# cwchenwang/outdoor-nerf-depth

Hardware: AMD Instinct MI355X
Metric: train rays/sec, KITTI 375x1242, 64+128 samples/ray (higher is better)
Workload: dtype bf16 MFMA operands, f32 accumulate / f32 master weights

## Files before the change

include/nerfpp_hip.h:

```cpp
#ifndef NERFPP_HIP_H
#define NERFPP_HIP_H

#include <stdint.h>

#ifdef __cplusplus
extern "C" {
#endif

#define NERFPP_ABI_VERSION 9

#define NERFPP_OK 0
#define NERFPP_ERR_ARG 1
#define NERFPP_ERR_HIP 2
#define NERFPP_ERR_INTERNAL 3
#define NERFPP_ERR_UNSUPPORTED 4
#define NERFPP_ERR_COMM 5
#define NERFPP_ERR_LAUNCH NERFPP_ERR_HIP

#define NERFPP_PREC_BF16 1
#define NERFPP_PREC_SPLIT_BF16 2
#define NERFPP_PREC_FP16X2W 3

#define NERFPP_LOSS_RGB_ONLY 0
#define NERFPP_LOSS_MSE 1
#define NERFPP_LOSS_L1 2
#define NERFPP_LOSS_KL 3

#define NERFPP_FG_PARAMS 595844
#define NERFPP_BG_PARAMS 606596
#define NERFPP_LEVEL_PARAMS 1202440
#define NERFPP_MAX_SAMPLES 256

const char* nerfpp_last_error(void);
int nerfpp_abi_version(void);


int nerfpp_intersect_sphere(void* stream, int n_rays, const float* ray_o, const float* ray_d,
                            float* fg_far, int* bad_count);

int nerfpp_sample_coarse(void* stream, int n_rays, int n_samples, const float* ray_o,
                         const float* ray_d, const float* min_depth, const float* t_rand_fg,
                         const float* t_rand_bg, float* fg_far, float* fg_z, float* bg_z,
                         int* bad_count);

int nerfpp_sample_coarse_rng(void* stream, int n_rays, int n_samples, const float* ray_o,
                             const float* ray_d, const float* min_depth, uint64_t seed, uint64_t step,
                             float* fg_far, float* fg_z, float* bg_z, int* bad_count);

int nerfpp_rng_uniform(void* stream, uint64_t seed, uint64_t step, int stream_id, int64_t n, float* out);

int nerfpp_perturb_samples(void* stream, int n_rays, int n_samples, const float* z_vals,
                           const float* t_rand, float* out);

int nerfpp_sample_pdf(void* stream, int n_rays, int n_bins_m, int n_new, const float* bins,
                      const float* weights, const float* u, float* samples, int64_t* above_inds);

int nerfpp_sample_fine(void* stream, int n_rays, int s_old, int n_new, const float* z_old,
                       const float* weights, const float* u, float* z_merged, float* samples,
                       int64_t* above_inds);

int nerfpp_sample_fine_pair(void* stream, int n_rays, int s_old, int n_new, const float* fg_z_old,
                            const float* fg_weights, const float* fg_u, float* fg_z_merged,
                            const float* bg_z_old, const float* bg_weights, const float* bg_u,
                            float* bg_z_merged);

int nerfpp_sample_fine_pair_rng(void* stream, int n_rays, int s_old, int n_new, const float* fg_z_old,
                                const float* fg_weights, float* fg_z_merged, const float* bg_z_old,
                                const float* bg_weights, float* bg_z_merged, uint64_t seed, uint64_t step);

int nerfpp_sample_pixels(void* stream, uint64_t seed, uint64_t step, int64_t n_pixels, int n_rays, int64_t* pix);

int nerfpp_gather_rays(void* stream, int n_rays, int width, const float* cam, const int64_t* pix,
                       const float* rgb_img, const float* depth_img, float* ray_o, float* ray_d,
                       float* rgb, float* depth_sup, float* min_depth);


int nerfpp_table_sizes(int net, int64_t* fwd_elems, int64_t* fwd_bias_elems, int64_t* bwd_elems,
                       int64_t* slab_floats, int64_t* n_params);
int nerfpp_build_tables(int net, int32_t* fwd_tbl, int32_t* bias_tbl, int32_t* bwd_tbl,
                        int32_t* unpack_tbl);
int64_t nerfpp_level_tables_elems(void);
int nerfpp_build_level_tables(int32_t* host_tables);

int nerfpp_dw_plan(int64_t rows, int backward_precision, int32_t* k_out, int32_t* is_full_out);

int64_t nerfpp_packed_bytes(int precision);
int nerfpp_pack_level(void* stream, int precision, const float* params, const int32_t* tables,
                      void* packed);


int64_t nerfpp_workspace_bytes(int n_rays, int n_samples, int precision, int training);

int nerfpp_workspace_tensor(int n_rays, int n_samples, int precision, int net, int tensor,
                            int64_t* byte_offset, int32_t* ld, int64_t* plane_bytes);

typedef struct {
  int32_t n_rays, n_samples;
  int32_t precision, training;
  const float* ray_o;
  const float* ray_d;
  const float* fg_far;
  const float* fg_z;
  const float* bg_z;
  const void* packed;
  void* workspace;
  float* rgb;
  float* depth;
  float* fg_weights;
  float* bg_weights;
  float* fg_dists;
  float* fg_rgb;
  float* fg_depth;
  float* bg_rgb;
  float* bg_depth;
  float* bg_lambda;
  void* ev_mlp_begin;
  void* ev_mlp_end;
} nerfpp_forward_args;

int nerfpp_level_forward(void* stream, const nerfpp_forward_args* args);

int nerfpp_loss(void* stream, int n_rays, int n_samples, int loss_type, float lambda_depth,
                float kl_sigma, const float* rgb, const float* rgb_gt, const float* depth,
                const float* depth_sup, const float* fg_weights, const float* fg_z,
                const float* fg_dists, const float* fg_far, float* scalars, float* g_rgb,
                float* g_depth, float* g_fg_weights);

typedef struct {
  int32_t n_rays, n_samples;
  int32_t precision;
  int32_t workspace_precision;
  const float* ray_d;
  const float* fg_far;
  const float* fg_z;
  const float* bg_z;
  const void* packed;
  void* workspace;
  const int32_t* tables;
  const float* g_rgb;
  const float* g_depth;
  const float* g_fg_weights;
  float grad_scale;
  float* grads;
  void* ev_bwd_begin;
  void* ev_bwd_end;
  void* ev_dw_begin;
  void* ev_dw_end;
  const float* params;
  int32_t defer_reduce;
  int32_t fused_loss;
  int32_t loss_type;
  float lambda_depth;
  float kl_sigma;
  const float* rgb;
  const float* depth;
  const float* rgb_gt;
  const float* depth_sup;
  const int32_t* bad_count;
} nerfpp_backward_args;

int nerfpp_level_backward(void* stream, const nerfpp_backward_args* args);

int nerfpp_level_reduce_grads(void* stream, const nerfpp_backward_args* args);

int nerfpp_adam_step(void* stream, float* params, const float* grads, float* exp_avg,
                     float* exp_avg_sq, int64_t n, int step, double lr, double beta1, double beta2,
                     double eps, const float* skip_if_nonzero);

const char* nerfpp_comm_last_error(void);
int nerfpp_rccl_unique_id(char out_id[128]);
int nerfpp_rccl_comm_init(void** comm, int world_size, const char id[128], int rank);
int nerfpp_rccl_comm_destroy(void* comm);
int nerfpp_allreduce_mean(void* stream, void* rccl_comm, float* grads, int64_t count, int world_size, int prescaled);

int64_t nerfpp_image_metrics_workspace_bytes(int n_frames, int H, int W);
int nerfpp_image_metrics_u8(void* stream, int n_frames, int H, int W, const uint8_t* gt, const uint8_t* pred,
                            void* workspace, double* out);

#ifdef __cplusplus
}
#endif
#endif
```

outdoor_nerf_depth_amd/_lib.py:

```python
import ctypes as C
import os

from . import _ctypes_util as U

_HERE = os.path.dirname(os.path.abspath(__file__))
LIB_PATH = os.environ.get('NERFPP_HIP_LIB') or os.path.join(_HERE, 'libnerfpp_hip.so')

OK = 0
ABI_VERSION = 9
PREC_BF16, PREC_SPLIT_BF16 = 1, 2
PREC_FP16_FWD = 3
PREC_SPLIT_FWD = 12
LOSS_RGB_ONLY, LOSS_MSE, LOSS_L1, LOSS_KL = 0, 1, 2, 3
LOSS_TYPES = {'rgbonly': LOSS_RGB_ONLY, 'mse': LOSS_MSE, 'l1': LOSS_L1, 'kl': LOSS_KL}
FG_PARAMS, BG_PARAMS, LEVEL_PARAMS = 595844, 606596, 1202440
MAX_SAMPLES = 256

_fp = C.c_void_p
_i64p = C.POINTER(C.c_int64)
_i32p = C.POINTER(C.c_int32)


class ForwardArgs(C.Structure):
    _fields_ = [('n_rays', C.c_int32), ('n_samples', C.c_int32), ('precision', C.c_int32),
                ('training', C.c_int32)] + \
               [(k, _fp) for k in ('ray_o', 'ray_d', 'fg_far', 'fg_z', 'bg_z', 'packed', 'workspace',
                                   'rgb', 'depth', 'fg_weights', 'bg_weights', 'fg_dists', 'fg_rgb',
                                   'fg_depth', 'bg_rgb', 'bg_depth', 'bg_lambda', 'ev_mlp_begin',
                                   'ev_mlp_end')]


class BackwardArgs(C.Structure):
    _fields_ = [('n_rays', C.c_int32), ('n_samples', C.c_int32), ('precision', C.c_int32),
                ('workspace_precision', C.c_int32)] + \
               [(k, _fp) for k in ('ray_d', 'fg_far', 'fg_z', 'bg_z', 'packed', 'workspace', 'tables',
                                   'g_rgb', 'g_depth', 'g_fg_weights')] + \
               [('grad_scale', C.c_float), ('grads', _fp)] + \
               [(k, _fp) for k in ('ev_bwd_begin', 'ev_bwd_end', 'ev_dw_begin', 'ev_dw_end', 'params')] + \
               [('defer_reduce', C.c_int32), ('fused_loss', C.c_int32), ('loss_type', C.c_int32),
                ('lambda_depth', C.c_float), ('kl_sigma', C.c_float)] + \
               [(k, _fp) for k in ('rgb', 'depth', 'rgb_gt', 'depth_sup', 'bad_count')]


SYMBOLS = {
    'nerfpp_last_error': (C.c_char_p, []),
    'nerfpp_abi_version': (C.c_int, []),
    'nerfpp_intersect_sphere': (C.c_int, [_fp, C.c_int, _fp, _fp, _fp, _fp]),
    'nerfpp_sample_coarse': (C.c_int, [_fp, C.c_int, C.c_int] + [_fp] * 9),
    'nerfpp_sample_coarse_rng': (C.c_int, [_fp, C.c_int, C.c_int, _fp, _fp, _fp, C.c_uint64, C.c_uint64, _fp, _fp, _fp, _fp]),
    'nerfpp_rng_uniform': (C.c_int, [_fp, C.c_uint64, C.c_uint64, C.c_int, C.c_int64, _fp]),
    'nerfpp_sample_pixels': (C.c_int, [_fp, C.c_uint64, C.c_uint64, C.c_int64, C.c_int, _fp]),
    'nerfpp_perturb_samples': (C.c_int, [_fp, C.c_int, C.c_int, _fp, _fp, _fp]),
    'nerfpp_sample_pdf': (C.c_int, [_fp, C.c_int, C.c_int, C.c_int, _fp, _fp, _fp, _fp, _fp]),
    'nerfpp_sample_fine': (C.c_int, [_fp, C.c_int, C.c_int, C.c_int, _fp, _fp, _fp, _fp, _fp, _fp]),
    'nerfpp_sample_fine_pair': (C.c_int, [_fp, C.c_int, C.c_int, C.c_int, _fp, _fp, _fp, _fp, _fp, _fp, _fp, _fp]),
    'nerfpp_sample_fine_pair_rng': (C.c_int, [_fp, C.c_int, C.c_int, C.c_int, _fp, _fp, _fp, _fp, _fp, _fp, C.c_uint64,
                                              C.c_uint64]),
    'nerfpp_gather_rays': (C.c_int, [_fp, C.c_int, C.c_int] + [_fp] * 9),
    'nerfpp_table_sizes': (C.c_int, [C.c_int, _i64p, _i64p, _i64p, _i64p, _i64p]),
    'nerfpp_build_tables': (C.c_int, [C.c_int, _i32p, _i32p, _i32p, _i32p]),
    'nerfpp_level_tables_elems': (C.c_int64, []),
    'nerfpp_build_level_tables': (C.c_int, [_i32p]),
    'nerfpp_dw_plan': (C.c_int, [C.c_int64, C.c_int, _i32p, _i32p]),
    'nerfpp_packed_bytes': (C.c_int64, [C.c_int]),
    'nerfpp_pack_level': (C.c_int, [_fp, C.c_int, _fp, _fp, _fp]),
    'nerfpp_workspace_bytes': (C.c_int64, [C.c_int, C.c_int, C.c_int, C.c_int]),
    'nerfpp_workspace_tensor': (C.c_int, [C.c_int, C.c_int, C.c_int, C.c_int, C.c_int, _i64p, _i32p, _i64p]),
    'nerfpp_level_forward': (C.c_int, [_fp, C.POINTER(ForwardArgs)]),
    'nerfpp_loss': (C.c_int, [_fp, C.c_int, C.c_int, C.c_int, C.c_float, C.c_float] + [_fp] * 12),
    'nerfpp_level_backward': (C.c_int, [_fp, C.POINTER(BackwardArgs)]),
    'nerfpp_level_reduce_grads': (C.c_int, [_fp, C.POINTER(BackwardArgs)]),
    'nerfpp_adam_step': (C.c_int, [_fp, _fp, _fp, _fp, _fp, C.c_int64, C.c_int, C.c_double, C.c_double,
                                   C.c_double, C.c_double, _fp]),
    'nerfpp_image_metrics_workspace_bytes': (C.c_int64, [C.c_int, C.c_int, C.c_int]),
    'nerfpp_image_metrics_u8': (C.c_int, [_fp, C.c_int, C.c_int, C.c_int, _fp, _fp, _fp, _fp]),
    'nerfpp_comm_last_error': (C.c_char_p, []),
    'nerfpp_rccl_unique_id': (C.c_int, [C.c_char_p]),
    'nerfpp_rccl_comm_init': (C.c_int, [C.POINTER(C.c_void_p), C.c_int, C.c_char_p, C.c_int]),
    'nerfpp_rccl_comm_destroy': (C.c_int, [_fp]),
    'nerfpp_allreduce_mean': (C.c_int, [_fp, _fp, _fp, C.c_int64, C.c_int, C.c_int]),
}

_lib = None


class NerfppError(RuntimeError):
    pass


def lib():
    global _lib
    if _lib is None:
        _lib = U.load(LIB_PATH, 'libnerfpp_hip.so', SYMBOLS, 'nerfpp_abi_version', ABI_VERSION, NerfppError,
                      ' (hipcc --offload-arch=gfx950). There is no CPU fallback for the NeRF++ hot path.')
    return _lib


check = U.checker(lib, 'nerfpp_last_error', NerfppError, 'nerfpp call')


def build_level_tables():
    import numpy as np
    n = lib().nerfpp_level_tables_elems()
    out = np.empty(n, np.int32)
    check(lib().nerfpp_build_level_tables(out.ctypes.data_as(_i32p)), 'nerfpp_build_level_tables')
    return out


def build_net_tables(net):
    import numpy as np
    sizes = [C.c_int64() for _ in range(5)]
    check(lib().nerfpp_table_sizes(net, *[C.byref(s) for s in sizes]), 'nerfpp_table_sizes')
    fwd, bias, bwd, slab, npar = [s.value for s in sizes]
    arrs = [np.empty(n, np.int32) for n in (fwd, bias, bwd, npar)]
    check(lib().nerfpp_build_tables(net, *[a.ctypes.data_as(_i32p) for a in arrs]), 'nerfpp_build_tables')
    return arrs[0], arrs[1], arrs[2], arrs[3], slab
```

outdoor_nerf_depth_amd/csrc/nerfpp_api.hip:

```cpp
#include "probe_env.h"
#include <hip/hip_runtime.h>
#include <stdio.h>
#include <stdlib.h>
#include <string.h>
#include "../../include/nerfpp_hip.h"
#define API_OK NERFPP_OK
#define API_ERR_HIP NERFPP_ERR_HIP
#define API_ERR_ARG NERFPP_ERR_ARG
#include "api_common.h"
#include "nerfpp_common.h"
#include "nerfpp_kernels.h"

using namespace nerfpp;

namespace {

constexpr size_t align_up(size_t v, size_t a) { return (v + a - 1) / a * a; }
bool h0_recomputed(int WP) { return a_planes(WP) == 1; }

struct TblLayout { int64_t fwd[2], bias[2], bwd[2], unpack[2], total; };
TblLayout tbl_layout() {
  TblLayout L{};
  int64_t off = 0;
  for (int net = 0; net < N_NET; ++net) {
    L.fwd[net] = off; off += (int64_t)fwd_frags(net) * 512;
    L.bias[net] = off; off += FWD_BIAS_FLOATS;
    L.bwd[net] = off; off += (int64_t)BWD_FRAGS * 512;
    L.unpack[net] = off; off += net_params(net);
  }
  L.total = off;
  return L;
}

struct PackLayout { size_t fwd[2], bwd[2], bias[2], derived[2], total; };
PackLayout pack_layout(int P) {
  PackLayout L{};
  size_t off = 0;
  for (int net = 0; net < N_NET; ++net) {
    L.fwd[net] = off; off = align_up(off + fwd_stream_bytes(net, P), 256);
    L.bwd[net] = off; off = align_up(off + bwd_stream_bytes(P), 256);
    L.bias[net] = off; off = align_up(off + FWD_BIAS_FLOATS * sizeof(float), 256);
    L.derived[net] = off; off = align_up(off + DERIVED_FLOATS * sizeof(float), 256);
  }
  L.total = off;
  return L;
}

struct WsLayout {
  size_t tensor[2][T_COUNT], out_raw[2], depth_real, d_out[2], slabs[2], masks[2], fix_m[2], total;
  int64_t rows, rows_padded;
  int ksplit;
};
int choose_ksplit(int64_t rows) {
  int k = 1;
  for (int rc = 0; rc < 2; ++rc) {
    const DwPlan pl = dw_plan(rows, rc != 0);
    for (int net = 0; net < N_NET; ++net)
      for (int j = 0; j < DW_JOBS; ++j) k = pl.k[net][j] > k ? pl.k[net][j] : k;
  }
  return k;
}
WsLayout ws_layout(int n_rays, int S, int P, bool training) {
  WsLayout L{};
  L.rows = (int64_t)n_rays * S;
  L.rows_padded = (int64_t)align_up((size_t)L.rows, 256);
  L.ksplit = choose_ksplit(L.rows);
  size_t off = 0;
  for (int net = 0; net < N_NET; ++net) {
    L.out_raw[net] = off; off = align_up(off + (size_t)L.rows_padded * 16, 256);
    if (training) {
      L.d_out[net] = off; off = align_up(off + (size_t)L.rows_padded * 16, 256);
      for (int t = 0; t < T_COUNT; ++t) {
        L.tensor[net][t] = off;
        if (t == T_R || t == T_DR) continue;
        if (t == T_DG) continue;
        if (t == T_H0 && h0_recomputed(P)) continue;
        if (t == T_DZ0 + 7 && h0_recomputed(P)) continue;
        off = align_up(off + (size_t)L.rows_padded * tensor_ld(net, t) * 2 * a_planes(P), 256);
      }
      L.slabs[net] = off; off = align_up(off + (size_t)L.ksplit * gslab_floats(net) * 4, 256);
      L.masks[net] = off; off = align_up(off + (size_t)9 * (L.rows_padded / 32) * 64 * 16, 256);
      L.fix_m[net] = off; off = align_up(off + (size_t)128 * 256 * 4, 256);
    }
  }
  L.depth_real = off; off = align_up(off + (size_t)L.rows_padded * 4, 256);
  L.total = off;
  return L;
}

NetWs make_netws(char* ws, const WsLayout& L, int net) {
  NetWs w;
  for (int t = 0; t < T_COUNT; ++t) w.t[t] = (__bf16*)(ws + L.tensor[net][t]);
  w.t[T_DG] = w.t[T_DS] + (DG_COL0 / 16) * (FRAG_BYTES / 2);
  return w;
}

bool prec_ok(int P) { return P == NERFPP_PREC_BF16 || P == NERFPP_PREC_SPLIT_BF16; }
bool prec_ok_fwd(int P) { return prec_ok(P) || P == NERFPP_PREC_FP16X2W; }

bool split_nets() {
  static const bool on = PROBE_GETENV("NERFPP_MLP_SPLIT") != nullptr;
  return on;
}

}

extern "C" {

const char* nerfpp_last_error(void) { return g_err; }
int nerfpp_abi_version(void) { return NERFPP_ABI_VERSION; }

int nerfpp_intersect_sphere(void* stream, int n_rays, const float* ray_o, const float* ray_d, float* fg_far,
                            int* bad_count) {
  REQUIRE(n_rays > 0 && ray_o && ray_d && fg_far, "non-null inputs, n_rays > 0");
  launch_intersect_sphere((hipStream_t)stream, n_rays, ray_o, ray_d, fg_far, bad_count);
  return check_launch("intersect_sphere");
}

int nerfpp_sample_coarse(void* stream, int n_rays, int n_samples, const float* ray_o, const float* ray_d,
                         const float* min_depth, const float* t_rand_fg, const float* t_rand_bg, float* fg_far,
                         float* fg_z, float* bg_z, int* bad_count) {
  REQUIRE(n_rays > 0 && n_samples >= 2 && n_samples <= NERFPP_MAX_SAMPLES, "2 <= n_samples <= 256");
  REQUIRE(ray_o && ray_d && min_depth && fg_far && fg_z && bg_z, "non-null pointers");
  launch_sample_coarse((hipStream_t)stream, n_rays, n_samples, ray_o, ray_d, min_depth, t_rand_fg, t_rand_bg,
                       fg_far, fg_z, bg_z, bad_count, make_rng_key(0, 0, false));
  return check_launch("sample_coarse");
}

int nerfpp_sample_coarse_rng(void* stream, int n_rays, int n_samples, const float* ray_o, const float* ray_d,
                             const float* min_depth, uint64_t seed, uint64_t step, float* fg_far, float* fg_z,
                             float* bg_z, int* bad_count) {
  REQUIRE(n_rays > 0 && n_samples >= 2 && n_samples <= NERFPP_MAX_SAMPLES, "2 <= n_samples <= 256");
  REQUIRE(ray_o && ray_d && min_depth && fg_far && fg_z && bg_z, "non-null pointers");
  launch_sample_coarse((hipStream_t)stream, n_rays, n_samples, ray_o, ray_d, min_depth, nullptr, nullptr, fg_far,
                       fg_z, bg_z, bad_count, make_rng_key(seed, step, true));
  return check_launch("sample_coarse_rng");
}

int nerfpp_rng_uniform(void* stream, uint64_t seed, uint64_t step, int stream_id, int64_t n, float* out) {
  REQUIRE(n > 0 && out && stream_id >= 0 && stream_id <= 3, "stream_id in 0..3, non-null output");
  launch_rng_uniform((hipStream_t)stream, make_rng_key(seed, step, true), (uint32_t)stream_id, n, out);
  return check_launch("rng_uniform");
}

int nerfpp_perturb_samples(void* stream, int n_rays, int n_samples, const float* z_vals, const float* t_rand,
                           float* out) {
  REQUIRE(n_rays > 0 && n_samples >= 2 && z_vals && t_rand && out, "non-null pointers");
  launch_perturb((hipStream_t)stream, n_rays, n_samples, z_vals, t_rand, out);
  return check_launch("perturb_samples");
}

int nerfpp_sample_pdf(void* stream, int n_rays, int n_bins_m, int n_new, const float* bins, const float* weights,
                      const float* u, float* samples, int64_t* above_inds) {
  REQUIRE(n_rays > 0 && n_bins_m >= 1 && n_bins_m + 1 <= 512 && n_new >= 1 && n_new <= 512, "sizes");
  REQUIRE(bins && weights && samples, "non-null pointers");
  launch_sample_pdf((hipStream_t)stream, false, n_rays, n_bins_m, n_new, bins, weights, u, samples, above_inds,
                    nullptr);
  return check_launch("sample_pdf");
}

int nerfpp_sample_fine(void* stream, int n_rays, int s_old, int n_new, const float* z_old, const float* weights,
                       const float* u, float* z_merged, float* samples, int64_t* above_inds) {
  REQUIRE(n_rays > 0 && s_old >= 3 && n_new >= 1 && s_old + n_new <= 512, "3 <= s_old, s_old + n_new <= 512");
  REQUIRE(z_old && weights && z_merged, "non-null pointers");
  launch_sample_pdf((hipStream_t)stream, true, n_rays, s_old - 2, n_new, z_old, weights, u, samples, above_inds,
                    z_merged);
  return check_launch("sample_fine");
}

int nerfpp_sample_fine_pair(void* stream, int n_rays, int s_old, int n_new, const float* fg_z_old,
                            const float* fg_weights, const float* fg_u, float* fg_z_merged, const float* bg_z_old,
                            const float* bg_weights, const float* bg_u, float* bg_z_merged) {
  REQUIRE(n_rays > 0 && s_old >= 3 && n_new >= 1 && s_old + n_new <= 512, "3 <= s_old, s_old + n_new <= 512");
  REQUIRE(fg_z_old && fg_weights && fg_z_merged && bg_z_old && bg_weights && bg_z_merged, "non-null pointers");
  const float* z[2] = {fg_z_old, bg_z_old};
  const float* w[2] = {fg_weights, bg_weights};
  const float* u[2] = {fg_u, bg_u};
  float* m[2] = {fg_z_merged, bg_z_merged};
  launch_sample_fine_pair((hipStream_t)stream, n_rays, s_old - 2, n_new, z, w, u, m, make_rng_key(0, 0, false));
  return check_launch("sample_fine_pair");
}

int nerfpp_sample_fine_pair_rng(void* stream, int n_rays, int s_old, int n_new, const float* fg_z_old,
                                const float* fg_weights, float* fg_z_merged, const float* bg_z_old,
                                const float* bg_weights, float* bg_z_merged, uint64_t seed, uint64_t step) {
  REQUIRE(n_rays > 0 && s_old >= 3 && n_new >= 1 && s_old + n_new <= 512, "3 <= s_old, s_old + n_new <= 512");
  REQUIRE(fg_z_old && fg_weights && fg_z_merged && bg_z_old && bg_weights && bg_z_merged, "non-null pointers");
  const float* z[2] = {fg_z_old, bg_z_old};
  const float* w[2] = {fg_weights, bg_weights};
  const float* u[2] = {nullptr, nullptr};
  float* m[2] = {fg_z_merged, bg_z_merged};
  launch_sample_fine_pair((hipStream_t)stream, n_rays, s_old - 2, n_new, z, w, u, m, make_rng_key(seed, step, true));
  return check_launch("sample_fine_pair_rng");
}

int nerfpp_sample_pixels(void* stream, uint64_t seed, uint64_t step, int64_t n_pixels, int n_rays, int64_t* pix) {
  REQUIRE(pix && n_rays >= 1 && n_rays <= 8192, "1 <= n_rays <= 8192, non-null output");
  REQUIRE(n_pixels >= n_rays && n_pixels < ((int64_t)1 << 31), "n_rays <= n_pixels < 2^31");
  launch_sample_pixels((hipStream_t)stream, make_rng_key(seed, step, true), n_pixels, n_rays, pix);
  return check_launch("sample_pixels");
}

int nerfpp_gather_rays(void* stream, int n_rays, int width, const float* cam, const int64_t* pix,
                       const float* rgb_img, const float* depth_img, float* ray_o, float* ray_d, float* rgb,
                       float* depth_sup, float* min_depth) {
  REQUIRE(n_rays > 0 && width > 0 && cam && pix && ray_o && ray_d && min_depth, "non-null pointers");
  REQUIRE((rgb == nullptr) || rgb_img, "rgb output needs rgb_img");
  REQUIRE((depth_sup == nullptr) || depth_img, "depth_sup output needs depth_img");
  launch_gather_rays((hipStream_t)stream, n_rays, width, cam, pix, rgb_img, depth_img, ray_o, ray_d, rgb, depth_sup,
                     min_depth);
  return check_launch("gather_rays");
}

int64_t nerfpp_level_tables_elems(void) { return tbl_layout().total; }

int nerfpp_build_level_tables(int32_t* host_tables) {
  if (!host_tables) return fail(NERFPP_ERR_ARG, "nerfpp_build_level_tables: null buffer");
  const TblLayout L = tbl_layout();
  for (int net = 0; net < N_NET; ++net) {
    const int rc = nerfpp_build_tables(net, host_tables + L.fwd[net], host_tables + L.bias[net],
                                       host_tables + L.bwd[net], host_tables + L.unpack[net]);
    if (rc != NERFPP_OK) return fail(rc, "nerfpp_build_tables(%d) failed", net);
  }
  return NERFPP_OK;
}

int nerfpp_dw_plan(int64_t rows, int backward_precision, int32_t* k_out, int32_t* is_full_out) {
  if (!k_out || rows <= 0 || !prec_ok(backward_precision)) return -1;
  const DwPlan pl = dw_plan(rows, backward_precision == 1);
  const JobTable jt = build_all_jobs();
  for (int net = 0; net < N_NET; ++net)
    for (int j = 0; j < DW_JOBS; ++j) {
      k_out[net * DW_JOBS + j] = pl.k[net][j];
      if (is_full_out) is_full_out[net * DW_JOBS + j] = dw_job_is_full(jt.jobs[net][j]) ? 1 : 0;
    }
  return DW_JOBS;
}

int64_t nerfpp_packed_bytes(int precision) { return prec_ok_fwd(precision) ? (int64_t)pack_layout(precision).total : -1; }

int nerfpp_pack_level(void* stream, int precision, const float* params, const int32_t* tables, void* packed) {
  REQUIRE(prec_ok_fwd(precision), "precision must be 1, 2 or 3");
  REQUIRE(params && tables && packed, "non-null pointers");
  const TblLayout T = tbl_layout();
  const PackLayout L = pack_layout(precision);
  hipStream_t st = (hipStream_t)stream;
  char* out = (char*)packed;
  const int32_t* tbl[3 * N_NET];
  void* outs[3 * N_NET];
  int64_t n[3 * N_NET];
  for (int net = 0; net < N_NET; ++net) {
    tbl[3 * net] = tables + T.fwd[net];      outs[3 * net] = out + L.fwd[net];      n[3 * net] = (int64_t)fwd_frags(net) * 512;
    tbl[3 * net + 1] = tables + T.bwd[net];  outs[3 * net + 1] = out + L.bwd[net];  n[3 * net + 1] = (int64_t)BWD_FRAGS * 512;
    tbl[3 * net + 2] = tables + T.bias[net]; outs[3 * net + 2] = out + L.bias[net]; n[3 * net + 2] = FWD_BIAS_FLOATS;
  }
  float* derived[N_NET] = {(float*)(out + L.derived[0]), (float*)(out + L.derived[1])};
  launch_pack_level(st, params, precision, tbl, outs, n, derived);
  return check_launch("pack_level");
}

int64_t nerfpp_workspace_bytes(int n_rays, int n_samples, int precision, int training) {
  if (n_rays <= 0 || n_samples < 2 || n_samples > NERFPP_MAX_SAMPLES || !prec_ok_fwd(precision)) return -1;
  return (int64_t)ws_layout(n_rays, n_samples, precision, training != 0).total;
}

int nerfpp_workspace_tensor(int n_rays, int n_samples, int precision, int net, int tensor, int64_t* byte_offset,
                            int32_t* ld, int64_t* plane_bytes) {
  REQUIRE(n_rays > 0 && n_samples >= 2 && n_samples <= NERFPP_MAX_SAMPLES && prec_ok_fwd(precision), "sizes / precision");
  REQUIRE(net >= 0 && net < N_NET && tensor >= 0 && tensor < T_COUNT && tensor != T_R && tensor != T_DR, "net / tensor id");
  REQUIRE(byte_offset && ld && plane_bytes, "non-null outputs");
  if (tensor == T_H0 && h0_recomputed(precision))
    return fail(NERFPP_ERR_UNSUPPORTED, "nerfpp_workspace_tensor: H0 is not materialised at precision %d (its weight-gradient job recomputes it from X)", precision);
  if (tensor == T_DZ0 + 7 && h0_recomputed(precision))
    return fail(NERFPP_ERR_UNSUPPORTED, "nerfpp_workspace_tensor: dZ7 is not materialised at precision %d (its weight-gradient job recomputes it from [dS | dG])", precision);
  const WsLayout L = ws_layout(n_rays, n_samples, precision, true);
  const int l = tensor_ld(net, tensor);
  *byte_offset = tensor == T_DG ? (int64_t)L.tensor[net][T_DS] + (DG_COL0 / 16) * FRAG_BYTES : (int64_t)L.tensor[net][tensor];
  *ld = l;
  *plane_bytes = (int64_t)L.rows_padded * l * 2;
  return NERFPP_OK;
}

int nerfpp_level_forward(void* stream, const nerfpp_forward_args* a) {
  REQUIRE(a, "args");
  REQUIRE(a->n_rays > 0 && a->n_samples >= 2 && a->n_samples <= NERFPP_MAX_SAMPLES, "sizes");
  REQUIRE(prec_ok_fwd(a->precision), "precision must be 1, 2 or 3");
  REQUIRE(a->ray_o && a->ray_d && a->fg_far && a->fg_z && a->bg_z && a->packed && a->workspace, "inputs");
  REQUIRE(a->rgb && a->depth && a->fg_weights && a->bg_weights && a->fg_dists && a->fg_rgb && a->fg_depth &&
          a->bg_rgb && a->bg_depth && a->bg_lambda, "outputs");
  hipStream_t st = (hipStream_t)stream;
  const int P = a->precision;
  const bool train = a->training != 0;
  const WsLayout L = ws_layout(a->n_rays, a->n_samples, P, train);
  const PackLayout PL = pack_layout(P);
  char* ws = (char*)a->workspace;
  const char* pk = (const char*)a->packed;
  MlpFwdArgs mm[N_NET];
  for (int net = 0; net < N_NET; ++net) {
    MlpFwdArgs& m = mm[net];
    m = MlpFwdArgs{};
    m.geom.ray_o = a->ray_o;
    m.geom.ray_d = a->ray_d;
    m.geom.z = net == 0 ? a->fg_z : a->bg_z;
    m.rows = L.rows;
    m.rows_padded = L.rows_padded;
    m.S = a->n_samples;
    m.w_stream = pk + PL.fwd[net];
    m.bias = (const float*)(pk + PL.bias[net]);
    m.out_raw = (float*)(ws + L.out_raw[net]);
    m.depth_real = (float*)(ws + L.depth_real);
    if (train) { m.ws = make_netws(ws, L, net); m.masks = (uint4*)(ws + L.masks[net]); }
    m.save_lo = a->training == 2 ? 0 : 1;
    m.skip_h0 = (train && (h0_recomputed(P) || a->training == 2)) ? 1 : 0;
  }
  if (a->ev_mlp_begin) (void)hipEventRecord((hipEvent_t)a->ev_mlp_begin, st);
  if (split_nets()) {
    launch_mlp_fwd_pair(st, P, train, mm[0], mm[1], 1);
    launch_mlp_fwd_pair(st, P, train, mm[0], mm[1], 2);
  } else {
    launch_mlp_fwd_pair(st, P, train, mm[0], mm[1], 0);
  }
  if (a->ev_mlp_end) (void)hipEventRecord((hipEvent_t)a->ev_mlp_end, st);
  launch_composite_fwd(st, a->n_rays, a->n_samples, (const float*)(ws + L.out_raw[0]),
                       (const float*)(ws + L.out_raw[1]), (const float*)(ws + L.depth_real), a->ray_d, a->fg_far,
                       a->fg_z, a->bg_z, a->rgb, a->depth, a->fg_weights, a->bg_weights, a->fg_dists, a->fg_rgb,
                       a->fg_depth, a->bg_rgb, a->bg_depth, a->bg_lambda);
  return check_launch("level_forward");
}

int nerfpp_loss(void* stream, int n_rays, int n_samples, int loss_type, float lambda_depth, float kl_sigma,
                const float* rgb, const float* rgb_gt, const float* depth, const float* depth_sup,
                const float* fg_weights, const float* fg_z, const float* fg_dists, const float* fg_far,
                float* scalars, float* g_rgb, float* g_depth, float* g_fg_weights) {
  REQUIRE(n_rays > 0 && loss_type >= 0 && loss_type <= 3, "loss_type in 0..3");
  REQUIRE(rgb && rgb_gt && scalars && g_rgb && g_depth, "non-null pointers");
  if (loss_type != NERFPP_LOSS_RGB_ONLY) REQUIRE(depth && depth_sup, "depth loss needs depth and depth_sup");
  if (loss_type == NERFPP_LOSS_KL)
    REQUIRE(fg_weights && fg_z && fg_dists && fg_far && g_fg_weights && kl_sigma > 0.f, "KL inputs");
  launch_loss((hipStream_t)stream, n_rays, n_samples, loss_type, lambda_depth, kl_sigma, rgb, rgb_gt, depth,
              depth_sup, fg_weights, fg_z, fg_dists, fg_far, scalars, g_rgb, g_depth, g_fg_weights);
  return check_launch("loss");
}

}

static void weight_grads(hipStream_t st, const nerfpp_backward_args* a, const WsLayout& L) {
  char* ws = (char*)a->workspace;
  DwArgs dw{};
  for (int net = 0; net < N_NET; ++net) {
    dw.ws[net] = make_netws(ws, L, net);
    dw.slabs[net] = (float*)(ws + L.slabs[net]);
  }
  dw.rows = L.rows;
  dw.rows_padded = L.rows_padded;
  dw.h0_from_x = a->precision == 1 ? 1 : 0;
  const PackLayout PL = pack_layout(a->precision);
  for (int net = 0; net < N_NET; ++net) {
    dw.fwd_w[net] = (const char*)a->packed + PL.fwd[net];
    dw.fwd_bias[net] = (const float*)((const char*)a->packed + PL.bias[net]);
    dw.bwd_w[net] = (const char*)a->packed + PL.bwd[net];
    dw.masks[net] = (const uint4*)(ws + L.masks[net]);
  }
  dw.plan = dw_plan(L.rows, dw.h0_from_x != 0);
  if (a->ev_dw_begin) (void)hipEventRecord((hipEvent_t)a->ev_dw_begin, st);
  launch_dw(st, a->precision, dw);
  if (a->ev_dw_end) (void)hipEventRecord((hipEvent_t)a->ev_dw_end, st);
}
static bool defer_dw() {
  static const bool on = PROBE_GETENV("NERFPP_DEFER_DW") != nullptr;
  return on;
}

static void reduce_grads(hipStream_t st, const nerfpp_backward_args* a, const WsLayout& L, const TblLayout& T) {
  char* ws = (char*)a->workspace;
  const DwPlan plan = dw_plan(L.rows, a->precision == 1);
  const float* slabs[N_NET];
  int64_t slab_floats[N_NET];
  const int32_t* utbl[N_NET];
  float* m_out[N_NET];
  for (int net = 0; net < N_NET; ++net) {
    slabs[net] = (const float*)(ws + L.slabs[net]);
    slab_floats[net] = gslab_floats(net);
    utbl[net] = a->tables + T.unpack[net];
    m_out[net] = (float*)(ws + L.fix_m[net]);
  }
  static const int skip = PROBE_GETENV("NERFPP_REDUCE_SKIP") ? atoi(PROBE_GETENV("NERFPP_REDUCE_SKIP")) : 0;
  if (!(skip & 1)) launch_unpack_grads(st, slabs, slab_floats, plan, utbl, m_out, a->grad_scale, a->grads, a->bad_count);
  if (!(skip & 2)) launch_remap_fixup(st, a->grads, a->params, m_out[0], m_out[1]);
}

extern "C" {

int nerfpp_level_reduce_grads(void* stream, const nerfpp_backward_args* a) {
  REQUIRE(a, "args");
  REQUIRE(a->n_rays > 0 && a->n_samples >= 2 && a->n_samples <= NERFPP_MAX_SAMPLES, "sizes");
  REQUIRE(prec_ok(a->precision), "precision must be 1 or 2");
  REQUIRE(a->workspace && a->tables && a->grads && a->params, "workspace / tables / grads / params");
  const int WP = a->workspace_precision ? a->workspace_precision : a->precision;
  REQUIRE(prec_ok_fwd(WP) && a_planes(WP) >= a_planes(a->precision), "workspace_precision: 0, or a forward precision that saved the planes this backward reads");
  const WsLayout L = ws_layout(a->n_rays, a->n_samples, WP, true);
  if (defer_dw()) weight_grads((hipStream_t)stream, a, L);
  reduce_grads((hipStream_t)stream, a, L, tbl_layout());
  return check_launch("level_reduce_grads");
}

int nerfpp_level_backward(void* stream, const nerfpp_backward_args* a) {
  REQUIRE(a, "args");
  REQUIRE(a->n_rays > 0 && a->n_samples >= 2 && a->n_samples <= NERFPP_MAX_SAMPLES, "sizes");
  REQUIRE(prec_ok(a->precision), "precision must be 1 or 2");
  REQUIRE(a->ray_d && a->fg_far && a->fg_z && a->bg_z && a->packed && a->workspace && a->tables, "inputs");
  REQUIRE(a->grads && a->params, "gradients / params");
  LossFuse lf{};
  if (a->fused_loss) {
    REQUIRE(a->loss_type >= NERFPP_LOSS_RGB_ONLY && a->loss_type <= NERFPP_LOSS_KL, "loss_type in 0..3");
    REQUIRE(a->rgb && a->rgb_gt, "fused loss head needs rgb and rgb_gt");
    if (a->loss_type != NERFPP_LOSS_RGB_ONLY) REQUIRE(a->depth && a->depth_sup, "fused depth loss needs depth and depth_sup");
    if (a->loss_type == NERFPP_LOSS_KL) REQUIRE(a->kl_sigma > 0.f, "kl_sigma > 0");
    lf.type = a->loss_type; lf.lambda_depth = a->lambda_depth; lf.kl_sigma = a->kl_sigma;
    lf.rgb = a->rgb; lf.depth = a->depth; lf.rgb_gt = a->rgb_gt; lf.depth_sup = a->depth_sup;
  } else {
    REQUIRE(a->g_rgb && a->g_depth, "dL/d rgb and dL/d depth (or fused_loss)");
  }
  hipStream_t st = (hipStream_t)stream;
  const int P = a->precision;
  const int WP = a->workspace_precision ? a->workspace_precision : P;
  REQUIRE(prec_ok_fwd(WP) && a_planes(WP) >= a_planes(P), "workspace_precision: 0, or a forward precision that saved the planes this backward reads");
  const WsLayout L = ws_layout(a->n_rays, a->n_samples, WP, true);
  const PackLayout PL = pack_layout(P);
  const TblLayout T = tbl_layout();
  char* ws = (char*)a->workspace;
  const char* pk = (const char*)a->packed;
  launch_composite_bwd(st, a->n_rays, a->n_samples, (const float*)(ws + L.out_raw[0]),
                       (const float*)(ws + L.out_raw[1]), (const float*)(ws + L.depth_real), a->ray_d, a->fg_far,
                       a->fg_z, a->bg_z, a->g_rgb, a->g_depth, a->g_fg_weights, (float*)(ws + L.d_out[0]),
                       (float*)(ws + L.d_out[1]), a->fused_loss ? &lf : nullptr);
  MlpBwdArgs mb[N_NET];
  for (int net = 0; net < N_NET; ++net) {
    MlpBwdArgs& m = mb[net];
    m = MlpBwdArgs{};
    m.rows = L.rows;
    m.rows_padded = L.rows_padded;
    m.w_stream = pk + PL.bwd[net];
    m.d_out = (const float*)(ws + L.d_out[net]);
    m.ws = make_netws(ws, L, net);
    m.masks = (const uint4*)(ws + L.masks[net]);
    m.skip_dz7 = P == 1 ? 1 : 0;
  }
  if (a->ev_bwd_begin) (void)hipEventRecord((hipEvent_t)a->ev_bwd_begin, st);
  if (split_nets()) {
    launch_mlp_bwd_pair(st, P, mb[0], mb[1], 1);
    launch_mlp_bwd_pair(st, P, mb[0], mb[1], 2);
  } else {
    launch_mlp_bwd_pair(st, P, mb[0], mb[1], 0);
  }
  if (a->ev_bwd_end) (void)hipEventRecord((hipEvent_t)a->ev_bwd_end, st);
  if (!(a->defer_reduce && defer_dw())) weight_grads(st, a, L);
  if (!a->defer_reduce) reduce_grads(st, a, L, T);
  return check_launch("level_backward");
}

int nerfpp_adam_step(void* stream, float* params, const float* grads, float* exp_avg, float* exp_avg_sq,
                     int64_t n, int step, double lr, double beta1, double beta2, double eps,
                     const float* skip_if_nonzero) {
  REQUIRE(params && grads && exp_avg && exp_avg_sq && n > 0 && step >= 1, "non-null pointers, step >= 1");
  launch_adam((hipStream_t)stream, params, grads, exp_avg, exp_avg_sq, n, step, lr, beta1, beta2, eps, skip_if_nonzero);
  return check_launch("adam_step");
}

static int image_metrics_sizes_ok(const char* fn, int n_frames, int H, int W) {
  if (n_frames < 1 || n_frames > 65535) return fail(NERFPP_ERR_ARG, "%s: n_frames = %d, expected 1 .. 65535", fn, n_frames);
  if (H < 7 || W < 7)
    return fail(NERFPP_ERR_ARG, "%s: a %d x %d image is smaller than the 7 x 7 SSIM window (H >= 7 and W >= 7)", fn, H, W);
  if (H > 32768 || W > 32768) return fail(NERFPP_ERR_ARG, "%s: a %d x %d image exceeds 32768 pixels per side", fn, H, W);
  return NERFPP_OK;
}

int64_t nerfpp_image_metrics_workspace_bytes(int n_frames, int H, int W) {
  if (image_metrics_sizes_ok(__func__, n_frames, H, W) != NERFPP_OK) return -1;
  return (int64_t)n_frames * image_metrics_tiles(H, W) * 4 * 8;
}

int nerfpp_image_metrics_u8(void* stream, int n_frames, int H, int W, const uint8_t* gt, const uint8_t* pred,
                            void* workspace, double* out) {
  const int rc = image_metrics_sizes_ok(__func__, n_frames, H, W);
  if (rc != NERFPP_OK) return rc;
  REQUIRE(gt && pred && workspace && out, "non-null gt, pred, workspace, out");
  REQUIRE(((uintptr_t)workspace & 7) == 0 && ((uintptr_t)out & 7) == 0, "workspace and out aligned to 8 bytes");
  launch_image_metrics((hipStream_t)stream, n_frames, H, W, gt, pred, workspace, out);
  return check_launch("image_metrics_u8");
}

}
```

outdoor_nerf_depth_amd/csrc/nerfpp_kernels.h:

```cpp
#pragma once
#include <hip/hip_runtime.h>
#include <stdint.h>
#include "nerfpp_common.h"

namespace nerfpp {

struct MlpGeom {
  const float* ray_o;
  const float* ray_d;
  const float* z;
};

struct NetWs {
  __bf16* t[T_COUNT];
};

struct MlpFwdArgs {
  MlpGeom geom;
  int64_t rows, rows_padded;
  int S;
  const void* w_stream;
  const float* bias;
  float* out_raw;
  float* depth_real;
  NetWs ws;
  uint4* masks;
  int save_lo;
  int skip_h0;
};

struct MlpBwdArgs {
  int64_t rows, rows_padded;
  const void* w_stream;
  const float* d_out;
  NetWs ws;
  const uint4* masks;
  int skip_dz7;
};

struct LossFuse {
  int type;
  float lambda_depth, kl_sigma;
  const float* rgb;
  const float* depth;
  const float* rgb_gt;
  const float* depth_sup;
};

struct DwArgs {
  NetWs ws[N_NET];
  int64_t rows, rows_padded;
  float* slabs[N_NET];
  DwPlan plan;
  int h0_from_x;
  const void* fwd_w[N_NET];
  const float* fwd_bias[N_NET];
  const void* bwd_w[N_NET];
  const uint4* masks[N_NET];
};

}

void launch_intersect_sphere(hipStream_t st, int n, const float* o, const float* d, float* far, int* bad);
void launch_sample_coarse(hipStream_t st, int n, int S, const float* o, const float* d, const float* min_depth,
                          const float* t_fg, const float* t_bg, float* far, float* fg_z, float* bg_z, int* bad,
                          const nerfpp::RngKey& rng);
void launch_rng_uniform(hipStream_t st, const nerfpp::RngKey& rng, uint32_t stream_id, int64_t n, float* out);
void launch_perturb(hipStream_t st, int n, int S, const float* z, const float* t, float* out);
void launch_sample_pdf(hipStream_t st, bool fused, int n, int M, int S_new, const float* bins_or_zold,
                       const float* weights, const float* u, float* samples, int64_t* above, float* merged);
void launch_sample_fine_pair(hipStream_t st, int n, int M, int S_new, const float* const* z_old,
                             const float* const* weights, const float* const* u, float* const* merged,
                             const nerfpp::RngKey& rng);
void launch_composite_fwd(hipStream_t st, int n, int S, const float* raw_fg, const float* raw_bg,
                          const float* depth_real_bg, const float* ray_d, const float* fg_far,
                          const float* fg_z, const float* bg_z, float* rgb, float* depth, float* fg_weights,
                          float* bg_weights, float* fg_dists, float* fg_rgb, float* fg_depth, float* bg_rgb,
                          float* bg_depth, float* bg_lambda);
void launch_composite_bwd(hipStream_t st, int n, int S, const float* raw_fg, const float* raw_bg,
                          const float* depth_real_bg, const float* ray_d, const float* fg_far,
                          const float* fg_z, const float* bg_z, const float* g_rgb, const float* g_depth,
                          const float* g_fg_weights, float* dout_fg, float* dout_bg, const nerfpp::LossFuse* lf);
void launch_loss(hipStream_t st, int n, int S, int type, float lambda_depth, float kl_sigma, const float* rgb,
                 const float* rgb_gt, const float* depth, const float* depth_sup, const float* fg_weights,
                 const float* fg_z, const float* fg_dists, const float* fg_far, float* scalars, float* g_rgb,
                 float* g_depth, float* g_fg_weights);
int launch_sample_pixels(hipStream_t st, const nerfpp::RngKey& rng, int64_t n_pixels, int k, int64_t* pix);
void launch_gather_rays(hipStream_t st, int n, int W, const float* cam, const int64_t* pix, const float* rgb_img,
                        const float* depth_img, float* ray_o, float* ray_d, float* rgb, float* depth_sup,
                        float* min_depth);
void launch_mlp_fwd_pair(hipStream_t st, int P, bool train, const nerfpp::MlpFwdArgs& a_fg, const nerfpp::MlpFwdArgs& a_bg, int which);
void launch_mlp_bwd_pair(hipStream_t st, int P, const nerfpp::MlpBwdArgs& a_fg, const nerfpp::MlpBwdArgs& a_bg, int which);
void launch_dw(hipStream_t st, int P, const nerfpp::DwArgs& a);
void launch_pack_level(hipStream_t st, const float* params, int P, const int32_t* const* tbl, void* const* out,
                       const int64_t* n, float* const* derived);
void launch_unpack_grads(hipStream_t st, const float* const* slabs, const int64_t* slab_floats,
                         const nerfpp::DwPlan& plan, const int32_t* const* tbl, float* const* m_out, float scale,
                         float* grads_lvl, const int32_t* bad_count);
void launch_remap_fixup(hipStream_t st, float* grads_lvl, const float* params_lvl, const float* m0, const float* m1);
void launch_adam(hipStream_t st, float* p, const float* g, float* m, float* v, int64_t n, int step, double lr,
                 double beta1, double beta2, double eps, const float* skip);
int64_t image_metrics_tiles(int H, int W);
void launch_image_metrics(hipStream_t st, int F, int H, int W, const unsigned char* gt, const unsigned char* pred,
                          void* workspace, double* out);
```

outdoor_nerf_depth_amd/csrc/nerfpp_render.hip:

```cpp
#include <hip/hip_runtime.h>
#include <math.h>
#include <stdint.h>
#include "hip_device.h"
#include "nerfpp_common.h"
#include "nerfpp_kernels.h"

namespace nerfpp {

using hipdev::wave_sum, hipdev::wave_excl_suffix_sum, hipdev::lds_tree_sum;

constexpr float TINY = 1e-6f;
constexpr float HUGE_NUM = 1e10f;

__device__ __forceinline__ float sum3(float a, float b, float c) { return (a + b) + c; }

__device__ __forceinline__ float sphere_far(const float* __restrict__ ray_o,
                                            const float* __restrict__ ray_d, int ray, int* bad) {
  const float ox = ray_o[ray * 3], oy = ray_o[ray * 3 + 1], oz = ray_o[ray * 3 + 2];
  const float dx = ray_d[ray * 3], dy = ray_d[ray * 3 + 1], dz = ray_d[ray * 3 + 2];
  const float dd = sum3(dx * dx, dy * dy, dz * dz);
  const float d1 = -sum3(dx * ox, dy * oy, dz * oz) / dd;
  const float px = ox + d1 * dx, py = oy + d1 * dy, pz = oz + d1 * dz;
  const float ray_d_cos = 1.f / sqrtf(dd);
  const float pn = sum3(px * px, py * py, pz * pz);
  if (pn >= 1.f && bad) atomicAdd(bad, 1);
  const float d2 = sqrtf(1.f - pn) * ray_d_cos;
  return d1 + d2;
}

__global__ void intersect_sphere_kernel(int n, const float* __restrict__ ray_o,
                                        const float* __restrict__ ray_d, float* __restrict__ far,
                                        int* bad) {
  const int ray = blockIdx.x * blockDim.x + threadIdx.x;
  if (ray < n) far[ray] = sphere_far(ray_o, ray_d, ray, bad);
}

__device__ __forceinline__ float torch_linspace01(int i, int steps) {
  const float step = 1.f / (float)(steps - 1);
  return i < steps / 2 ? fmaf(step, (float)i, 0.f) : fmaf(-step, (float)(steps - 1 - i), 1.f);
}

__device__ __forceinline__ float perturb(float zm, float z0, float zp, bool first, bool last, float t) {
  const float upper = last ? z0 : .5f * (zp + z0);
  const float lower = first ? z0 : .5f * (z0 + zm);
  return lower + (upper - lower) * t;
}

__global__ void sample_coarse_kernel(int n, int S, const float* __restrict__ ray_o,
                                     const float* __restrict__ ray_d,
                                     const float* __restrict__ min_depth,
                                     const float* __restrict__ t_fg, const float* __restrict__ t_bg,
                                     float* __restrict__ fg_far, float* __restrict__ fg_z,
                                     float* __restrict__ bg_z, int* bad, RngKey rng) {
  const int idx = blockIdx.x * blockDim.x + threadIdx.x;
  if (idx >= n * S) return;
  const int ray = idx / S, i = idx - ray * S;
  const float far = sphere_far(ray_o, ray_d, ray, i == 0 ? bad : nullptr);
  if (i == 0) fg_far[ray] = far;
  const float near = min_depth[ray];
  const float step = (far - near) / (float)(S - 1);
  const float z0 = near + (float)i * step;
  float out = z0;
  if (t_fg || rng.enabled) {
    const float zm = near + (float)(i - 1) * step, zp = near + (float)(i + 1) * step;
    out = perturb(zm, z0, zp, i == 0, i == S - 1, rng.enabled ? philox_uniform(rng, 0, (uint64_t)idx) : t_fg[idx]);
  }
  fg_z[idx] = out;
  const float b0 = torch_linspace01(i, S);
  out = b0;
  if (t_bg || rng.enabled) {
    const float bm = i > 0 ? torch_linspace01(i - 1, S) : 0.f;
    const float bp = i < S - 1 ? torch_linspace01(i + 1, S) : 0.f;
    out = perturb(bm, b0, bp, i == 0, i == S - 1, rng.enabled ? philox_uniform(rng, 1, (uint64_t)idx) : t_bg[idx]);
  }
  bg_z[idx] = out;
}

__global__ void rng_uniform_kernel(RngKey rng, uint32_t stream_id, int64_t n, float* __restrict__ out) {
  const int64_t i = (int64_t)blockIdx.x * blockDim.x + threadIdx.x;
  if (i < n) out[i] = philox_uniform(rng, stream_id, (uint64_t)i);
}

__global__ void perturb_kernel(int n, int S, const float* __restrict__ z, const float* __restrict__ t,
                               float* __restrict__ out) {
  const int idx = blockIdx.x * blockDim.x + threadIdx.x;
  if (idx >= n * S) return;
  const int i = idx % S;
  const float z0 = z[idx];
  const float zm = i > 0 ? z[idx - 1] : 0.f, zp = i < S - 1 ? z[idx + 1] : 0.f;
  out[idx] = perturb(zm, z0, zp, i == 0, i == S - 1, t[idx]);
}

constexpr int SP_MAX = 512;
__device__ __forceinline__ void lds_wave_sync() {
  asm volatile("s_waitcnt lgkmcnt(0)" ::: "memory");
  __builtin_amdgcn_wave_barrier();
}

struct SamplePdfProblem {
  const float* bins_or_zold; const float* weights; const float* u;
  float* samples; int64_t* above; float* merged;
};
struct SamplePdfArgs { SamplePdfProblem p[2]; RngKey rng; };
template <bool FUSED>
__global__ __launch_bounds__(256) void sample_pdf_kernel(int n, int M, int S_new, SamplePdfArgs args) {
  const SamplePdfProblem& pr = args.p[blockIdx.y];
  const float* __restrict__ bins_or_zold = pr.bins_or_zold;
  const float* __restrict__ weights = pr.weights;
  const float* __restrict__ u_in = pr.u;
  float* __restrict__ samples_out = pr.samples;
  int64_t* __restrict__ above_out = pr.above;
  float* __restrict__ merged_out = pr.merged;
  __shared__ float s_cdf[4][SP_MAX];
  __shared__ float s_w[4][SP_MAX];
  __shared__ float s_bins[4][SP_MAX];
  __shared__ float s_z[4][SP_MAX];
  const int wave = threadIdx.x >> 6, lane = threadIdx.x & 63;
  const int ray = blockIdx.x * 4 + wave;
  const bool active = ray < n;
  const int S_old = FUSED ? M + 2 : 0;
  float* cdf = s_cdf[wave];
  float* wq = s_w[wave];
  float* bins = s_bins[wave];
  float* zs = s_z[wave];
  if (active) {
    if (FUSED) {
      const float* zo = bins_or_zold + (size_t)ray * S_old;
      for (int i = lane; i < S_old; i += 64) zs[i] = zo[i];
      for (int k = lane; k < M; k += 64) wq[k] = weights[(size_t)ray * S_old + k + 1] + TINY;
    } else {
      for (int i = lane; i <= M; i += 64) bins[i] = bins_or_zold[(size_t)ray * (M + 1) + i];
      for (int k = lane; k < M; k += 64) wq[k] = weights[(size_t)ray * M + k] + TINY;
    }
  }
  __syncthreads();
  if (active) {
    if (FUSED)
      for (int i = lane; i <= M; i += 64) bins[i] = .5f * (zs[i + 1] + zs[i]);
    if (lane == 0) {
      double acc = 0.0;
      for (int k = 0; k < M; ++k) acc += (double)wq[k];
      cdf[0] = (float)acc;
    }
  }
  __syncthreads();
  if (active) {
    const float wsum = cdf[0];
    for (int k = lane; k < M; k += 64) wq[k] = wq[k] / wsum;
  }
  __syncthreads();
  if (active && lane == 0) {
    double acc = 0.0;
    cdf[0] = 0.f;
    for (int k = 0; k < M; ++k) {
      acc += (double)wq[k];
      cdf[k + 1] = (float)acc;
    }
  }
  __syncthreads();
  if (active) {
    for (int j = lane; j < S_new; j += 64) {
      const float u = args.rng.enabled ? philox_uniform(args.rng, 2u + blockIdx.y, (uint64_t)ray * S_new + j)
                      : u_in ? u_in[(size_t)ray * S_new + j] : torch_linspace01(j, S_new);
      int above = 0, hi_ = M;
      while (above < hi_) {
        const int mid = (above + hi_) >> 1;
        const bool ge = u >= cdf[mid];
        above = ge ? mid + 1 : above;
        hi_ = ge ? hi_ : mid;
      }
      const int below = above - 1 > 0 ? above - 1 : 0;
      const float cdf_lo = cdf[below], cdf_hi = cdf[above];
      const float bin_lo = bins[below], bin_hi = bins[above];
      float denom = cdf_hi - cdf_lo;
      denom = denom < TINY ? 1.f : denom;
      const float t = (u - cdf_lo) / denom;
      const float s = bin_lo + t * (bin_hi - bin_lo + TINY);
      if (samples_out) samples_out[(size_t)ray * S_new + j] = s;
      if (above_out) above_out[(size_t)ray * S_new + j] = above;
      if (FUSED) zs[S_old + j] = s;
    }
  }
  if (!FUSED) return;
  __syncthreads();
  if (active && merged_out) {
    const int S_tot = S_old + S_new;
    bool sorted_old = true;
    for (int i = lane; i + 1 < S_old; i += 64) sorted_old = sorted_old && zs[i] <= zs[i + 1];
    if (__all(sorted_old) && S_new <= SP_MAX) {
      int P2 = 1;
      while (P2 < S_new) P2 <<= 1;
      float* nb = wq;
      for (int i = lane; i < P2; i += 64) nb[i] = i < S_new ? zs[S_old + i] : __builtin_inff();
      lds_wave_sync();
      for (int k = 2; k <= P2; k <<= 1) {
        for (int j = k >> 1; j > 0; j >>= 1) {
          for (int t = lane; t < (P2 >> 1); t += 64) {
            const int lo = ((t & ~(j - 1)) << 1) | (t & (j - 1)), hi_i = lo | j;
            const bool up = (lo & k) == 0;
            const float x = nb[lo], y = nb[hi_i];
            if ((x > y) == up) { nb[lo] = y; nb[hi_i] = x; }
          }
          lds_wave_sync();
        }
      }
      float* mo = merged_out + (size_t)ray * S_tot;
      for (int i = lane; i < S_old; i += 64) {
        const float v = zs[i];
        int lo = 0, hi_i = S_new;
        while (lo < hi_i) {
          const int mid = (lo + hi_i) >> 1;
          const bool lt = nb[mid] < v;
          lo = lt ? mid + 1 : lo;
          hi_i = lt ? hi_i : mid;
        }
        mo[i + lo] = v;
      }
      for (int p = lane; p < S_new; p += 64) {
        const float v = nb[p];
        int lo = 0, hi_i = S_old;
        while (lo < hi_i) {
          const int mid = (lo + hi_i) >> 1;
          const bool le = zs[mid] <= v;
          lo = le ? mid + 1 : lo;
          hi_i = le ? hi_i : mid;
        }
        mo[p + lo] = v;
      }
      return;
    }
    if (S_tot <= 192) {
      const int e0 = lane, e1 = lane + 64, e2 = lane + 128;
      const float v0 = e0 < S_tot ? zs[e0] : 0.f, v1 = e1 < S_tot ? zs[e1] : 0.f, v2 = e2 < S_tot ? zs[e2] : 0.f;
      int r0 = 0, r1 = 0, r2 = 0;
#pragma unroll 4
      for (int k = 0; k < S_tot; ++k) {
        const float o = zs[k];
        r0 += (o < v0 || (o == v0 && k < e0)) ? 1 : 0;
        r1 += (o < v1 || (o == v1 && k < e1)) ? 1 : 0;
        r2 += (o < v2 || (o == v2 && k < e2)) ? 1 : 0;
      }
      float* mo = merged_out + (size_t)ray * S_tot;
      if (e0 < S_tot) mo[r0] = v0;
      if (e1 < S_tot) mo[r1] = v1;
      if (e2 < S_tot) mo[r2] = v2;
      return;
    }
    for (int e = lane; e < S_tot; e += 64) {
      const float v = zs[e];
      int rank = 0;
      for (int k = 0; k < S_tot; ++k) {
        const float o = zs[k];
        rank += (o < v || (o == v && k < e)) ? 1 : 0;
      }
      merged_out[(size_t)ray * S_tot + rank] = v;
    }
  }
}

constexpr int CPL_MAX = 4;

__device__ __forceinline__ float wave_excl_prod(float x, int lane, float* total) {
  float v = x;
#pragma unroll
  for (int d = 1; d < 64; d <<= 1) {
    const float t = __shfl_up(v, d, 64);
    if (lane >= d) v *= t;
  }
  *total = __shfl(v, 63, 64);
  const float e = __shfl_up(v, 1, 64);
  return lane == 0 ? 1.f : e;
}

struct RaySamples {
  float dist[CPL_MAX], e[CPL_MAX], alpha[CPL_MAX], q[CPL_MAX], T[CPL_MAX], w[CPL_MAX];
  float c[CPL_MAX][3], zval[CPL_MAX], sraw[CPL_MAX];
  float lambda;
};

template <bool BG>
__device__ __forceinline__ void load_volume(RaySamples& v, int S, int cpl, int lane, size_t row0,
                                            const float4* __restrict__ raw, const float* __restrict__ z,
                                            const float* __restrict__ depth_real, float dnorm, float far) {
  float run = 1.f;
#pragma unroll
  for (int k = 0; k < CPL_MAX; ++k) {
    const int i = lane * cpl + k;
    const bool ok = k < cpl && i < S;
    float dist = 0.f, sraw = 0.f, zv = 0.f;
    float c0 = 0.f, c1 = 0.f, c2 = 0.f;
    if (ok) {
      const int s = BG ? S - 1 - i : i;
      const float4 r = raw[row0 + s];
      c0 = r.x; c1 = r.y; c2 = r.z; sraw = r.w;
      if (BG) {
        const float zi = z[s];
        dist = i < S - 1 ? zi - z[s - 1] : HUGE_NUM;
        zv = depth_real[row0 + s];
      } else {
        const float zi = z[i];
        dist = dnorm * ((i < S - 1 ? z[i + 1] : far) - zi);
        zv = zi;
      }
    }
    const float sigma = fabsf(sraw);
    const float e = ok ? expf(-sigma * dist) : 1.f;
    const float alpha = 1.f - e;
    const float q = ok ? 1.f - alpha + TINY : 1.f;
    v.dist[k] = dist; v.e[k] = e; v.alpha[k] = alpha; v.q[k] = q;
    v.c[k][0] = c0; v.c[k][1] = c1; v.c[k][2] = c2; v.zval[k] = zv; v.sraw[k] = sraw;
    v.T[k] = run;
    run *= q;
  }
  float total;
  const float pre = wave_excl_prod(run, lane, &total);
  v.lambda = total;
#pragma unroll
  for (int k = 0; k < CPL_MAX; ++k) {
    v.T[k] *= pre;
    v.w[k] = v.alpha[k] * v.T[k];
  }
}

__global__ __launch_bounds__(256) void composite_fwd_kernel(
    int n, int S, const float4* __restrict__ raw_fg, const float4* __restrict__ raw_bg,
    const float* __restrict__ depth_real_bg, const float* __restrict__ ray_d,
    const float* __restrict__ fg_far, const float* __restrict__ fg_z, const float* __restrict__ bg_z,
    float* __restrict__ rgb, float* __restrict__ depth, float* __restrict__ fg_weights,
    float* __restrict__ bg_weights, float* __restrict__ fg_dists, float* __restrict__ fg_rgb,
    float* __restrict__ fg_depth, float* __restrict__ bg_rgb, float* __restrict__ bg_depth,
    float* __restrict__ bg_lambda) {
  const int wave = threadIdx.x >> 6, lane = threadIdx.x & 63;
  const int ray = blockIdx.x * 4 + wave;
  if (ray >= n) return;
  const int cpl = (S + 63) / 64;
  const size_t row0 = (size_t)ray * S;
  const float dx = ray_d[ray * 3], dy = ray_d[ray * 3 + 1], dz = ray_d[ray * 3 + 2];
  const float dnorm = sqrtf(sum3(dx * dx, dy * dy, dz * dz));
  RaySamples v;
  load_volume<false>(v, S, cpl, lane, row0, raw_fg, fg_z + row0, nullptr, dnorm, fg_far[ray]);
  float a0 = 0, a1 = 0, a2 = 0, ad = 0;
#pragma unroll
  for (int k = 0; k < CPL_MAX; ++k) {
    const int i = lane * cpl + k;
    if (k < cpl && i < S) {
      fg_weights[row0 + i] = v.w[k];
      fg_dists[row0 + i] = v.dist[k];
      a0 += v.w[k] * v.c[k][0]; a1 += v.w[k] * v.c[k][1]; a2 += v.w[k] * v.c[k][2];
      ad += v.w[k] * v.zval[k];
    }
  }
  const float f0 = wave_sum(a0), f1 = wave_sum(a1), f2 = wave_sum(a2), fd = wave_sum(ad);
  const float lam = v.lambda;
  load_volume<true>(v, S, cpl, lane, row0, raw_bg, bg_z + row0, depth_real_bg, dnorm, 0.f);
  a0 = a1 = a2 = ad = 0;
#pragma unroll
  for (int k = 0; k < CPL_MAX; ++k) {
    const int i = lane * cpl + k;
    if (k < cpl && i < S) {
      bg_weights[row0 + i] = v.w[k];
      a0 += v.w[k] * v.c[k][0]; a1 += v.w[k] * v.c[k][1]; a2 += v.w[k] * v.c[k][2];
      ad += v.w[k] * v.zval[k];
    }
  }
  const float b0 = lam * wave_sum(a0), b1 = lam * wave_sum(a1), b2 = lam * wave_sum(a2);
  const float bd = lam * wave_sum(ad);
  if (lane == 0) {
    fg_rgb[ray * 3] = f0; fg_rgb[ray * 3 + 1] = f1; fg_rgb[ray * 3 + 2] = f2;
    bg_rgb[ray * 3] = b0; bg_rgb[ray * 3 + 1] = b1; bg_rgb[ray * 3 + 2] = b2;
    rgb[ray * 3] = f0 + b0; rgb[ray * 3 + 1] = f1 + b1; rgb[ray * 3 + 2] = f2 + b2;
    fg_depth[ray] = fd; bg_depth[ray] = bd; depth[ray] = fd + bd; bg_lambda[ray] = lam;
  }
}

struct KlFuse { bool on; float gt, inv2s, lambda_depth; };
template <bool BG>
__device__ __forceinline__ void volume_backward(const RaySamples& v, int S, int cpl, int lane, size_t row0,
                                                const float gC[3], float gD, float g_lam_lam,
                                                const float* __restrict__ g_w_extra,
                                                float4* __restrict__ dout, const KlFuse kl = KlFuse{false, 0.f, 0.f, 0.f}) {
  float gw[CPL_MAX], term = 0.f;
#pragma unroll
  for (int k = 0; k < CPL_MAX; ++k) {
    const int i = lane * cpl + k;
    const bool ok = k < cpl && i < S;
    float g = gC[0] * v.c[k][0] + gC[1] * v.c[k][1] + gC[2] * v.c[k][2] + gD * v.zval[k];
    if (ok && g_w_extra) g += g_w_extra[row0 + i];
    if (!BG && ok && kl.on) {
      const float dz = v.zval[k] - kl.gt;
      const float w = v.w[k] + 1e-5f;
      const float e = expf(-(dz * dz) * kl.inv2s);
      g += -kl.lambda_depth * e * v.dist[k] / (w * (float)S);
    }
    gw[k] = ok ? g : 0.f;
    term += gw[k] * v.w[k];
  }
  float suffix = wave_excl_suffix_sum(term, lane);
#pragma unroll
  for (int k = CPL_MAX - 1; k >= 0; --k) {
    const int i = lane * cpl + k;
    if (k < cpl && i < S) {
      const float d_a = gw[k] * v.T[k] - (suffix + g_lam_lam) / v.q[k];
      const float d_sigma = d_a * v.dist[k] * v.e[k];
      const float sgn = v.sraw[k] > 0.f ? 1.f : (v.sraw[k] < 0.f ? -1.f : 0.f);
      float4 o;
      o.x = v.w[k] * gC[0] * v.c[k][0] * (1.f - v.c[k][0]);
      o.y = v.w[k] * gC[1] * v.c[k][1] * (1.f - v.c[k][1]);
      o.z = v.w[k] * gC[2] * v.c[k][2] * (1.f - v.c[k][2]);
      o.w = d_sigma * sgn;
      const int s = BG ? S - 1 - i : i;
      dout[row0 + s] = o;
    }
    suffix += gw[k] * v.w[k];
  }
}

template <bool LF>
__global__ __launch_bounds__(256) void composite_bwd_kernel(
    int n, int S, const float4* __restrict__ raw_fg, const float4* __restrict__ raw_bg,
    const float* __restrict__ depth_real_bg, const float* __restrict__ ray_d,
    const float* __restrict__ fg_far, const float* __restrict__ fg_z, const float* __restrict__ bg_z,
    const float* __restrict__ g_rgb, const float* __restrict__ g_depth,
    const float* __restrict__ g_fg_weights, float4* __restrict__ dout_fg, float4* __restrict__ dout_bg, LossFuse lf) {
  const int wave = threadIdx.x >> 6, lane = threadIdx.x & 63;
  const int ray = blockIdx.x * 4 + wave;
  float cnt = 0.f;
  if (LF && (lf.type == 1 || lf.type == 2)) {
    __shared__ float s_cnt[4];
    float c = 0.f;
    for (int r = threadIdx.x; r < n; r += 256) c += lf.depth_sup[r] > 0.f ? 1.f : 0.f;
    c = wave_sum(c);
    if (lane == 0) s_cnt[wave] = c;
    __syncthreads();
    cnt = (s_cnt[0] + s_cnt[1]) + (s_cnt[2] + s_cnt[3]);
  }
  if (ray >= n) return;
  const int cpl = (S + 63) / 64;
  const size_t row0 = (size_t)ray * S;
  const float dx = ray_d[ray * 3], dy = ray_d[ray * 3 + 1], dz = ray_d[ray * 3 + 2];
  const float dnorm = sqrtf(sum3(dx * dx, dy * dy, dz * dz));
  float gC[3], gD;
  KlFuse kl{false, 0.f, 0.f, 0.f};
  if (LF) {
#pragma unroll
    for (int c = 0; c < 3; ++c) gC[c] = 2.f * (lf.rgb[ray * 3 + c] - lf.rgb_gt[ray * 3 + c]) / (float)(3 * n);
    gD = 0.f;
    if (lf.type == 1 || lf.type == 2) {
      const float gt = lf.depth_sup[ray];
      if (gt > 0.f && cnt > 0.f) {
        const float d = lf.depth[ray] - gt;
        gD = lf.type == 1 ? lf.lambda_depth * 2.f * d / cnt
                          : lf.lambda_depth * (d > 0.f ? 1.f : (d < 0.f ? -1.f : 0.f)) / cnt;
      }
    } else if (lf.type == 3) {
      const float gt = lf.depth_sup[ray];
      kl.on = gt > 0.f && gt < fg_far[ray];
      kl.gt = gt;
      kl.inv2s = 1.f / (2.f * lf.kl_sigma);
      kl.lambda_depth = lf.lambda_depth;
    }
  } else {
    gC[0] = g_rgb[ray * 3]; gC[1] = g_rgb[ray * 3 + 1]; gC[2] = g_rgb[ray * 3 + 2];
    gD = g_depth[ray];
  }
  RaySamples vb;
  load_volume<true>(vb, S, cpl, lane, row0, raw_bg, bg_z + row0, depth_real_bg, dnorm, 0.f);
  float a0 = 0, a1 = 0, a2 = 0, ad = 0;
#pragma unroll
  for (int k = 0; k < CPL_MAX; ++k) {
    a0 += vb.w[k] * vb.c[k][0]; a1 += vb.w[k] * vb.c[k][1]; a2 += vb.w[k] * vb.c[k][2];
    ad += vb.w[k] * vb.zval[k];
  }
  const float g_lam = gC[0] * wave_sum(a0) + gC[1] * wave_sum(a1) + gC[2] * wave_sum(a2) + gD * wave_sum(ad);
  RaySamples vf;
  load_volume<false>(vf, S, cpl, lane, row0, raw_fg, fg_z + row0, nullptr, dnorm, fg_far[ray]);
  const float lam = vf.lambda;
  volume_backward<false>(vf, S, cpl, lane, row0, gC, gD, g_lam * lam, LF ? nullptr : g_fg_weights, dout_fg, kl);
  const float gCb[3] = {lam * gC[0], lam * gC[1], lam * gC[2]};
  volume_backward<true>(vb, S, cpl, lane, row0, gCb, lam * gD, 0.f, nullptr, dout_bg);
}

__device__ double block_sum(double v, double (&sh)[1][1024]) {
  lds_tree_sum(sh, {v});
  const double r = sh[0][0];
  __syncthreads();
  return r;
}

__global__ __launch_bounds__(256) void kl_terms_kernel(
    int n, int S, float lambda_depth, float kl_sigma, const float* __restrict__ depth_sup,
    const float* __restrict__ fg_weights, const float* __restrict__ fg_z, const float* __restrict__ fg_dists,
    const float* __restrict__ fg_far, float* __restrict__ ray_sum, float* __restrict__ g_fg_weights) {
  const int wave = threadIdx.x >> 6, lane = threadIdx.x & 63;
  const int ray = blockIdx.x * 4 + wave;
  if (ray >= n) return;
  const float gt = depth_sup[ray];
  const bool m = gt > 0.f && gt < fg_far[ray];
  const float inv2s = 1.f / (2.f * kl_sigma);
  double acc = 0.0;
  for (int s = lane; s < S; s += 64) {
    const size_t i = (size_t)ray * S + s;
    float g = 0.f;
    if (m) {
      const float dz = fg_z[i] - gt;
      const float w = fg_weights[i] + 1e-5f;
      const float e = expf(-(dz * dz) * inv2s);
      acc += (double)(-logf(w) * e * fg_dists[i]);
      g = -lambda_depth * e * fg_dists[i] / (w * (float)S);
    }
    g_fg_weights[i] = g;
  }
  acc = wave_sum(acc);
  if (lane == 0) ray_sum[ray] = (float)acc;
}

__global__ __launch_bounds__(1024) void loss_kernel(
    int n, int S, int type, float lambda_depth, float kl_sigma, const float* __restrict__ rgb,
    const float* __restrict__ rgb_gt, const float* __restrict__ depth, const float* __restrict__ depth_sup,
    const float* __restrict__ fg_weights, const float* __restrict__ fg_z, const float* __restrict__ fg_dists,
    const float* __restrict__ fg_far, float* __restrict__ scalars, float* __restrict__ g_rgb,
    float* __restrict__ g_depth, float* __restrict__ g_fg_weights) {
  __shared__ double sh[1][1024];
  double s_rgb = 0, s_dep = 0, s_cnt = 0;
  for (int r = threadIdx.x; r < n; r += blockDim.x) {
    for (int c = 0; c < 3; ++c) {
      const float d = rgb[r * 3 + c] - rgb_gt[r * 3 + c];
      s_rgb += (double)(d * d);
    }
    if (type == 0) continue;
    const float gt = depth_sup[r];
    if (type == 3) {
      const bool m = gt > 0.f && gt < fg_far[r];
      if (m) {
        s_cnt += 1;
        s_dep += (double)g_depth[r];
      }
    } else if (gt > 0.f) {
      const float d = gt - depth[r];
      s_cnt += 1;
      s_dep += type == 1 ? (double)(d * d) : (double)fabsf(d);
    }
  }
  const double t_rgb = block_sum(s_rgb, sh), t_dep = block_sum(s_dep, sh), t_cnt = block_sum(s_cnt, sh);
  const float rgb_loss = (float)(t_rgb / (3.0 * n));
  float depth_loss = 0.f;
  if (type == 3) depth_loss = (float)(t_dep / S);
  else if (type != 0) depth_loss = (float)(t_dep / t_cnt);
  if (threadIdx.x == 0) {
    scalars[0] = type == 0 ? rgb_loss : rgb_loss + lambda_depth * depth_loss;
    scalars[1] = rgb_loss;
    scalars[2] = depth_loss;
    scalars[3] = (float)t_cnt;
  }
  const float cnt = (float)t_cnt;
  for (int r = threadIdx.x; r < n; r += blockDim.x) {
    for (int c = 0; c < 3; ++c)
      g_rgb[r * 3 + c] = 2.f * (rgb[r * 3 + c] - rgb_gt[r * 3 + c]) / (float)(3 * n);
    float gd = 0.f;
    if (type == 1 || type == 2) {
      const float gt = depth_sup[r];
      if (gt > 0.f && cnt > 0.f) {
        const float d = depth[r] - gt;
        gd = type == 1 ? lambda_depth * 2.f * d / cnt
                       : lambda_depth * (d > 0.f ? 1.f : (d < 0.f ? -1.f : 0.f)) / cnt;
      }
    }
    g_depth[r] = gd;
    if (g_fg_weights && type != 3)
      for (int s = 0; s < S; ++s) g_fg_weights[(size_t)r * S + s] = 0.f;
  }
}

}

using namespace nerfpp;

void launch_intersect_sphere(hipStream_t st, int n, const float* o, const float* d, float* far, int* bad) {
  hipLaunchKernelGGL(intersect_sphere_kernel, dim3((n + 255) / 256), dim3(256), 0, st, n, o, d, far, bad);
}
void launch_sample_coarse(hipStream_t st, int n, int S, const float* o, const float* d, const float* min_depth,
                          const float* t_fg, const float* t_bg, float* far, float* fg_z, float* bg_z, int* bad,
                          const nerfpp::RngKey& rng) {
  const int tot = n * S;
  hipLaunchKernelGGL(sample_coarse_kernel, dim3((tot + 255) / 256), dim3(256), 0, st, n, S, o, d, min_depth,
                     t_fg, t_bg, far, fg_z, bg_z, bad, rng);
}
void launch_rng_uniform(hipStream_t st, const nerfpp::RngKey& rng, uint32_t stream_id, int64_t n, float* out) {
  hipLaunchKernelGGL(rng_uniform_kernel, dim3((unsigned)((n + 255) / 256)), dim3(256), 0, st, rng, stream_id, n, out);
}
void launch_perturb(hipStream_t st, int n, int S, const float* z, const float* t, float* out) {
  const int tot = n * S;
  hipLaunchKernelGGL(perturb_kernel, dim3((tot + 255) / 256), dim3(256), 0, st, n, S, z, t, out);
}
void launch_sample_pdf(hipStream_t st, bool fused, int n, int M, int S_new, const float* bins_or_zold,
                       const float* weights, const float* u, float* samples, int64_t* above, float* merged) {
  dim3 grid((n + 3) / 4), block(256);
  SamplePdfArgs a{};
  a.p[0] = SamplePdfProblem{bins_or_zold, weights, u, samples, above, merged};
  if (fused) hipLaunchKernelGGL(sample_pdf_kernel<true>, grid, block, 0, st, n, M, S_new, a);
  else hipLaunchKernelGGL(sample_pdf_kernel<false>, grid, block, 0, st, n, M, S_new, a);
}
void launch_sample_fine_pair(hipStream_t st, int n, int M, int S_new, const float* const* z_old,
                             const float* const* weights, const float* const* u, float* const* merged,
                             const nerfpp::RngKey& rng) {
  dim3 grid((n + 3) / 4, 2), block(256);
  SamplePdfArgs a{};
  a.rng = rng;
  for (int k = 0; k < 2; ++k) a.p[k] = SamplePdfProblem{z_old[k], weights[k], u[k], nullptr, nullptr, merged[k]};
  hipLaunchKernelGGL(sample_pdf_kernel<true>, grid, block, 0, st, n, M, S_new, a);
}
void launch_composite_fwd(hipStream_t st, int n, int S, const float* raw_fg, const float* raw_bg,
                          const float* depth_real_bg, const float* ray_d, const float* fg_far,
                          const float* fg_z, const float* bg_z, float* rgb, float* depth, float* fg_weights,
                          float* bg_weights, float* fg_dists, float* fg_rgb, float* fg_depth, float* bg_rgb,
                          float* bg_depth, float* bg_lambda) {
  hipLaunchKernelGGL(composite_fwd_kernel, dim3((n + 3) / 4), dim3(256), 0, st, n, S, (const float4*)raw_fg,
                     (const float4*)raw_bg, depth_real_bg, ray_d, fg_far, fg_z, bg_z, rgb, depth, fg_weights,
                     bg_weights, fg_dists, fg_rgb, fg_depth, bg_rgb, bg_depth, bg_lambda);
}
void launch_composite_bwd(hipStream_t st, int n, int S, const float* raw_fg, const float* raw_bg,
                          const float* depth_real_bg, const float* ray_d, const float* fg_far,
                          const float* fg_z, const float* bg_z, const float* g_rgb, const float* g_depth,
                          const float* g_fg_weights, float* dout_fg, float* dout_bg, const nerfpp::LossFuse* lf) {
  if (lf)
    hipLaunchKernelGGL(composite_bwd_kernel<true>, dim3((n + 3) / 4), dim3(256), 0, st, n, S, (const float4*)raw_fg,
                       (const float4*)raw_bg, depth_real_bg, ray_d, fg_far, fg_z, bg_z, g_rgb, g_depth,
                       g_fg_weights, (float4*)dout_fg, (float4*)dout_bg, *lf);
  else
    hipLaunchKernelGGL(composite_bwd_kernel<false>, dim3((n + 3) / 4), dim3(256), 0, st, n, S, (const float4*)raw_fg,
                       (const float4*)raw_bg, depth_real_bg, ray_d, fg_far, fg_z, bg_z, g_rgb, g_depth,
                       g_fg_weights, (float4*)dout_fg, (float4*)dout_bg, nerfpp::LossFuse{});
}
void launch_loss(hipStream_t st, int n, int S, int type, float lambda_depth, float kl_sigma, const float* rgb,
                 const float* rgb_gt, const float* depth, const float* depth_sup, const float* fg_weights,
                 const float* fg_z, const float* fg_dists, const float* fg_far, float* scalars, float* g_rgb,
                 float* g_depth, float* g_fg_weights) {
  if (type == 3)
    hipLaunchKernelGGL(kl_terms_kernel, dim3((n + 3) / 4), dim3(256), 0, st, n, S, lambda_depth, kl_sigma, depth_sup,
                       fg_weights, fg_z, fg_dists, fg_far, g_depth, g_fg_weights);
  hipLaunchKernelGGL(loss_kernel, dim3(1), dim3(1024), 0, st, n, S, type, lambda_depth, kl_sigma, rgb, rgb_gt,
                     depth, depth_sup, fg_weights, fg_z, fg_dists, fg_far, scalars, g_rgb, g_depth,
                     g_fg_weights);
}

namespace nerfpp {
__global__ void gather_rays_kernel(int n, int W, const float* __restrict__ cam, const int64_t* __restrict__ pix,
                                   const float* __restrict__ rgb_img, const float* __restrict__ depth_img,
                                   float* __restrict__ ray_o, float* __restrict__ ray_d, float* __restrict__ rgb,
                                   float* __restrict__ depth_sup, float* __restrict__ min_depth) {
  const int i = blockIdx.x * blockDim.x + threadIdx.x;
  if (i >= n) return;
  const int64_t p = pix[i];
  const float u = (float)(p % W) + 0.5f, v = (float)(p / W) + 0.5f;
  const float cx = (cam[0] * u + cam[1] * v) + cam[2];
  const float cy = (cam[3] * u + cam[4] * v) + cam[5];
  const float cz = (cam[6] * u + cam[7] * v) + cam[8];
  const float* c2w = cam + 9;
  ray_d[i * 3 + 0] = (c2w[0] * cx + c2w[1] * cy) + c2w[2] * cz;
  ray_d[i * 3 + 1] = (c2w[4] * cx + c2w[5] * cy) + c2w[6] * cz;
  ray_d[i * 3 + 2] = (c2w[8] * cx + c2w[9] * cy) + c2w[10] * cz;
  ray_o[i * 3 + 0] = c2w[3]; ray_o[i * 3 + 1] = c2w[7]; ray_o[i * 3 + 2] = c2w[11];
  if (rgb) { rgb[i * 3] = rgb_img[p * 3]; rgb[i * 3 + 1] = rgb_img[p * 3 + 1]; rgb[i * 3 + 2] = rgb_img[p * 3 + 2]; }
  if (depth_sup) depth_sup[i] = depth_img[p];
  min_depth[i] = 1e-4f;
}
}

namespace nerfpp {
constexpr int PIX_THREADS = 1024;
__global__ __launch_bounds__(PIX_THREADS) void sample_pixels_kernel(RngKey rng, uint32_t n, int k, int kp, int64_t* __restrict__ pix) {
  extern __shared__ __attribute__((aligned(16))) char pix_smem[];
  unsigned long long* keys = (unsigned long long*)pix_smem;
  uint32_t* x = (uint32_t*)(pix_smem + (size_t)kp * 8);
  uint32_t* ndraw = x + k;
  __shared__ int again;
  const uint32_t thresh = (0u - n) % n;
  auto draw = [&](int i) {
    uint32_t d = ndraw[i], v;
    for (;;) {
      const uint32_t w = philox_word(rng, 4u, (uint64_t)i + ((uint64_t)d << 20));
      ++d;
      const uint64_t m = (uint64_t)w * n;
      if ((uint32_t)m >= thresh) { v = (uint32_t)(m >> 32); break; }
    }
    ndraw[i] = d;
    x[i] = v;
  };
  for (int i = threadIdx.x; i < k; i += PIX_THREADS) { ndraw[i] = 0; draw(i); }
  for (;;) {
    __syncthreads();
    if (threadIdx.x == 0) again = 0;
    for (int i = threadIdx.x; i < kp; i += PIX_THREADS)
      keys[i] = i < k ? ((unsigned long long)x[i] << 32) | (unsigned)i : ~0ull;
    __syncthreads();
    for (int size = 2; size <= kp; size <<= 1)
      for (int stride = size >> 1; stride > 0; stride >>= 1) {
        for (int t = threadIdx.x; t < kp / 2; t += PIX_THREADS) {
          const int lo = 2 * t - (t & (stride - 1)), hi = lo + stride;
          const bool up = (lo & size) == 0;
          const unsigned long long a = keys[lo], b = keys[hi];
          if ((a > b) == up) { keys[lo] = b; keys[hi] = a; }
        }
        __syncthreads();
      }
    for (int p = threadIdx.x + 1; p < k; p += PIX_THREADS)
      if ((uint32_t)(keys[p] >> 32) == (uint32_t)(keys[p - 1] >> 32)) { draw((int)(uint32_t)keys[p]); again = 1; }
    __syncthreads();
    if (!again) break;
  }
  for (int i = threadIdx.x; i < k; i += PIX_THREADS) pix[i] = (int64_t)x[i];
}
}

int launch_sample_pixels(hipStream_t st, const nerfpp::RngKey& rng, int64_t n_pixels, int k, int64_t* pix) {
  int kp = 2;
  while (kp < k) kp <<= 1;
  const size_t lds = (size_t)kp * 8 + (size_t)k * 8;
  hipLaunchKernelGGL(nerfpp::sample_pixels_kernel, dim3(1), dim3(nerfpp::PIX_THREADS), lds, st, rng, (uint32_t)n_pixels, k, kp, pix);
  return 0;
}

void launch_gather_rays(hipStream_t st, int n, int W, const float* cam, const int64_t* pix, const float* rgb_img,
                        const float* depth_img, float* ray_o, float* ray_d, float* rgb, float* depth_sup,
                        float* min_depth) {
  hipLaunchKernelGGL(nerfpp::gather_rays_kernel, dim3((n + 255) / 256), dim3(256), 0, st, n, W, cam, pix, rgb_img,
                     depth_img, ray_o, ray_d, rgb, depth_sup, min_depth);
}
```

outdoor_nerf_depth_amd/ops.py:

```python
import ctypes as C
import functools
from collections import OrderedDict

import torch

from . import _ctypes_util as U
from . import _lib as L


_stream, _p = U.stream, U.p
_f32 = functools.partial(U.f32, error=L.NerfppError, fallback='the NeRF++ hot path has no CPU fallback')


def intersect_sphere(ray_o, ray_d):
    ray_o, ray_d = _f32(ray_o), _f32(ray_d)
    n = ray_o.shape[0]
    far = torch.empty(n, device=ray_o.device)
    bad = torch.zeros(1, dtype=torch.int32, device=ray_o.device)
    L.check(L.lib().nerfpp_intersect_sphere(_stream(), n, _p(ray_o), _p(ray_d), _p(far), _p(bad)),
            'nerfpp_intersect_sphere')
    if int(bad.item()) != 0:
        raise Exception(CAMERA_ERROR)
    return far


CAMERA_ERROR = ('Not all your cameras are bounded by the unit sphere; please make sure the '
                'cameras are normalized properly!')


def rng_uniform(seed, step, stream_id, shape, device):
    out = torch.empty(shape, device=device)
    L.check(L.lib().nerfpp_rng_uniform(_stream(), int(seed), int(step), int(stream_id), out.numel(), _p(out)),
            'nerfpp_rng_uniform')
    return out


def sample_pixels(n_pixels, n_rays, seed, step, device):
    pix = torch.empty(n_rays, dtype=torch.int64, device=device)
    L.check(L.lib().nerfpp_sample_pixels(_stream(), int(seed), int(step), int(n_pixels), int(n_rays), _p(pix)),
            'nerfpp_sample_pixels')
    return pix


def sample_coarse(ray_o, ray_d, min_depth, n_samples, t_rand_fg=None, t_rand_bg=None, perturb=True,
                  check=True, rng=None, bad=None):
    ray_o, ray_d, min_depth = _f32(ray_o), _f32(ray_d), _f32(min_depth)
    n = ray_o.shape[0]
    dev = ray_o.device
    if rng is not None and perturb:
        far = torch.empty(n, device=dev)
        fg_z = torch.empty(n, n_samples, device=dev)
        bg_z = torch.empty(n, n_samples, device=dev)
        if bad is None:
            bad = torch.zeros(1, dtype=torch.int32, device=dev)
        L.check(L.lib().nerfpp_sample_coarse_rng(_stream(), n, n_samples, _p(ray_o), _p(ray_d), _p(min_depth),
                                                 int(rng[0]), int(rng[1]), _p(far), _p(fg_z), _p(bg_z), _p(bad)),
                'nerfpp_sample_coarse_rng')
        if check and int(bad.item()) != 0:
            raise Exception(CAMERA_ERROR)
        return far, fg_z, bg_z
    if perturb:
        if t_rand_fg is None:
            t_rand_fg = torch.rand(n, n_samples, device=dev)
        if t_rand_bg is None:
            t_rand_bg = torch.rand(n, n_samples, device=dev)
        t_rand_fg, t_rand_bg = _f32(t_rand_fg, (n, n_samples)), _f32(t_rand_bg, (n, n_samples))
    else:
        t_rand_fg = t_rand_bg = None
    far = torch.empty(n, device=dev)
    fg_z = torch.empty(n, n_samples, device=dev)
    bg_z = torch.empty(n, n_samples, device=dev)
    if bad is None:
        bad = torch.zeros(1, dtype=torch.int32, device=dev)
    L.check(L.lib().nerfpp_sample_coarse(_stream(), n, n_samples, _p(ray_o), _p(ray_d), _p(min_depth),
                                         _p(t_rand_fg), _p(t_rand_bg), _p(far), _p(fg_z), _p(bg_z), _p(bad)),
            'nerfpp_sample_coarse')
    if check and int(bad.item()) != 0:
        raise Exception(CAMERA_ERROR)
    return far, fg_z, bg_z


def perturb_samples(z_vals, t_rand=None):
    z_vals = _f32(z_vals)
    if t_rand is None:
        t_rand = torch.rand_like(z_vals)
    t_rand = _f32(t_rand, z_vals.shape)
    out = torch.empty_like(z_vals)
    n, S = z_vals.shape
    L.check(L.lib().nerfpp_perturb_samples(_stream(), n, S, _p(z_vals), _p(t_rand), _p(out)),
            'nerfpp_perturb_samples')
    return out


def sample_pdf(bins, weights, N_samples, det=False, u=None, return_inds=False):
    bins, weights = _f32(bins), _f32(weights)
    n, M = weights.shape
    if bins.shape != (n, M + 1):
        raise L.NerfppError('bins must be [n, M+1]')
    if not det and u is None:
        u = torch.rand(n, N_samples, device=bins.device)
    u = None if det else _f32(u, (n, N_samples))
    samples = torch.empty(n, N_samples, device=bins.device)
    above = torch.empty(n, N_samples, dtype=torch.int64, device=bins.device) if return_inds else None
    L.check(L.lib().nerfpp_sample_pdf(_stream(), n, M, N_samples, _p(bins), _p(weights), _p(u), _p(samples),
                                      _p(above)), 'nerfpp_sample_pdf')
    return (samples, above) if return_inds else samples


def sample_fine(z_old, weights, N_samples, det=False, u=None, return_all=False):
    z_old, weights = _f32(z_old), _f32(weights)
    n, S_old = z_old.shape
    if weights.shape != (n, S_old):
        raise L.NerfppError('weights must be [n, S_old]')
    if not det and u is None:
        u = torch.rand(n, N_samples, device=z_old.device)
    u = None if det else _f32(u, (n, N_samples))
    merged = torch.empty(n, S_old + N_samples, device=z_old.device)
    samples = torch.empty(n, N_samples, device=z_old.device) if return_all else None
    above = torch.empty(n, N_samples, dtype=torch.int64, device=z_old.device) if return_all else None
    L.check(L.lib().nerfpp_sample_fine(_stream(), n, S_old, N_samples, _p(z_old), _p(weights), _p(u), _p(merged),
                                       _p(samples), _p(above)), 'nerfpp_sample_fine')
    return (merged, samples, above) if return_all else merged


def sample_fine_pair(fg_z, fg_weights, bg_z, bg_weights, N_samples, det=False, u_fg=None, u_bg=None, rng=None):
    fg_z, fg_weights, bg_z, bg_weights = _f32(fg_z), _f32(fg_weights), _f32(bg_z), _f32(bg_weights)
    n, S_old = fg_z.shape
    if fg_weights.shape != (n, S_old) or bg_z.shape != (n, S_old) or bg_weights.shape != (n, S_old):
        raise L.NerfppError('z / weights must all be [n, S_old]')
    if rng is not None and not det:
        fg_m = torch.empty(n, S_old + N_samples, device=fg_z.device)
        bg_m = torch.empty(n, S_old + N_samples, device=fg_z.device)
        L.check(L.lib().nerfpp_sample_fine_pair_rng(_stream(), n, S_old, N_samples, _p(fg_z), _p(fg_weights), _p(fg_m),
                                                    _p(bg_z), _p(bg_weights), _p(bg_m), int(rng[0]), int(rng[1])),
                'nerfpp_sample_fine_pair_rng')
        return fg_m, bg_m
    if det:
        u_fg = u_bg = None
    else:
        u_fg = _f32(u_fg, (n, N_samples)) if u_fg is not None else torch.rand(n, N_samples, device=fg_z.device)
        u_bg = _f32(u_bg, (n, N_samples)) if u_bg is not None else torch.rand(n, N_samples, device=fg_z.device)
    fg_m = torch.empty(n, S_old + N_samples, device=fg_z.device)
    bg_m = torch.empty(n, S_old + N_samples, device=fg_z.device)
    L.check(L.lib().nerfpp_sample_fine_pair(_stream(), n, S_old, N_samples, _p(fg_z), _p(fg_weights), _p(u_fg),
                                            _p(fg_m), _p(bg_z), _p(bg_weights), _p(u_bg), _p(bg_m)),
            'nerfpp_sample_fine_pair')
    return fg_m, bg_m


_TABLES = {}


def level_tables(device):
    key = str(device)
    if key not in _TABLES:
        _TABLES[key] = torch.from_numpy(L.build_level_tables()).to(device)
    return _TABLES[key]


RET_KEYS = ('rgb', 'fg_weights', 'bg_weights', 'fg_dists', 'fg_rgb', 'fg_depth', 'bg_rgb', 'bg_depth',
            'bg_lambda', 'depth')


class LevelEngine(object):

    def __init__(self, params_flat, precision=L.PREC_SPLIT_BF16):
        if params_flat.numel() != L.LEVEL_PARAMS:
            raise L.NerfppError('expected %d parameters, got %d' % (L.LEVEL_PARAMS, params_flat.numel()))
        self.params = _f32(params_flat)
        self.device = self.params.device
        precision = int(precision)
        if precision not in (L.PREC_BF16, L.PREC_SPLIT_BF16, L.PREC_FP16_FWD, L.PREC_SPLIT_FWD):
            raise L.NerfppError('unknown precision %r' % (precision,))
        self.precision = L.PREC_SPLIT_BF16 if precision == L.PREC_SPLIT_FWD else precision
        self.bwd_precision = L.PREC_BF16 if precision in (L.PREC_SPLIT_FWD, L.PREC_FP16_FWD) else precision
        self.tables = level_tables(self.device)
        self.packed = torch.empty(L.lib().nerfpp_packed_bytes(self.precision), dtype=torch.uint8,
                                  device=self.device)
        self.packed_bwd = self.packed if self.bwd_precision == self.precision else \
            torch.empty(L.lib().nerfpp_packed_bytes(self.bwd_precision), dtype=torch.uint8, device=self.device)
        self.workspace = None
        self._fwd = None
        self.repack()

    def repack(self):
        L.check(L.lib().nerfpp_pack_level(_stream(), self.precision, _p(self.params), _p(self.tables),
                                          _p(self.packed)), 'nerfpp_pack_level')
        if self.packed_bwd is not self.packed:
            L.check(L.lib().nerfpp_pack_level(_stream(), self.bwd_precision, _p(self.params), _p(self.tables),
                                              _p(self.packed_bwd)), 'nerfpp_pack_level')

    def _workspace(self, n, S, training):
        need = L.lib().nerfpp_workspace_bytes(n, S, self.precision, int(training))
        if need < 0:
            raise L.NerfppError('unsupported sizes n_rays=%d n_samples=%d' % (n, S))
        if self.workspace is None or self.workspace.numel() < need:
            self.workspace = torch.empty(need, dtype=torch.uint8, device=self.device)
        return self.workspace

    def forward(self, ray_o, ray_d, fg_z_max, fg_z_vals, bg_z_vals, training=False, events=None):
        ray_o, ray_d = _f32(ray_o), _f32(ray_d)
        n = ray_o.shape[0]
        fg_z_vals = _f32(fg_z_vals)
        S = fg_z_vals.shape[1]
        bg_z_vals, fg_z_max = _f32(bg_z_vals, (n, S)), _f32(fg_z_max, (n,))
        dev = self.device
        out = OrderedDict()
        for k in RET_KEYS:
            shape = (n, 3) if k in ('rgb', 'fg_rgb', 'bg_rgb') else \
                (n, S) if k in ('fg_weights', 'bg_weights', 'fg_dists') else (n,)
            out[k] = torch.empty(shape, device=dev)
        a = L.ForwardArgs()
        hi_only = training and self.bwd_precision != self.precision
        a.n_rays, a.n_samples, a.precision, a.training = n, S, self.precision, (2 if hi_only else int(training))
        a.ray_o, a.ray_d, a.fg_far, a.fg_z, a.bg_z = [t.data_ptr() for t in
                                                      (ray_o, ray_d, fg_z_max, fg_z_vals, bg_z_vals)]
        a.packed = self.packed.data_ptr()
        a.workspace = self._workspace(n, S, training).data_ptr()
        for k in RET_KEYS:
            setattr(a, k, out[k].data_ptr())
        if events is not None:
            a.ev_mlp_begin, a.ev_mlp_end = events[0].cuda_event, events[1].cuda_event
        L.check(L.lib().nerfpp_level_forward(_stream(), C.byref(a)), 'nerfpp_level_forward')
        if training:
            self._fwd = (n, S, ray_d, fg_z_max, fg_z_vals, bg_z_vals)
        return out

    def saved_tensor(self, net, tensor, plane=0):
        if self._fwd is None:
            raise L.NerfppError('saved_tensor() needs a preceding forward(training=True)')
        n, S = self._fwd[0], self._fwd[1]
        off, ld, pb = C.c_int64(), C.c_int32(), C.c_int64()
        L.check(L.lib().nerfpp_workspace_tensor(n, S, self.precision, int(net), int(tensor), C.byref(off), C.byref(ld),
                                                C.byref(pb)), 'nerfpp_workspace_tensor')
        rows, ld = n * S, ld.value
        rows_p = (rows + 31) // 32 * 32
        nblk = rows_p // 32 * (ld // 16)
        raw = self.workspace[off.value + plane * pb.value: off.value + plane * pb.value + nblk * 1024]
        blk = raw.view(torch.bfloat16).view(rows_p // 32, ld // 16, 32, 2, 8)
        blk = blk.view(rows_p // 32, ld // 16, 32, 2, 2, 4).permute(0, 2, 1, 4, 3, 5)
        return blk.reshape(rows_p, ld)[:rows].float()

    def backward(self, g_rgb, g_depth, g_fg_weights=None, grad_scale=1.0, out=None, events=None, defer_reduce=False,
                 fused_loss=None, bad_count=None):
        if self._fwd is None:
            raise L.NerfppError('backward() needs a preceding forward(training=True)')
        n, S, ray_d, fg_far, fg_z, bg_z = self._fwd
        keep = None
        if fused_loss is None:
            g_rgb, g_depth = _f32(g_rgb, (n, 3)), _f32(g_depth, (n,))
            g_fg_weights = _f32(g_fg_weights, (n, S)) if g_fg_weights is not None else None
        else:
            g_rgb = g_depth = g_fg_weights = None
            f = fused_loss
            t = L.LOSS_TYPES[f['loss_type']]
            keep = (_f32(f['ret']['rgb'], (n, 3)), _f32(f['ret']['depth'], (n,)), _f32(f['rgb_gt'], (n, 3)),
                    _f32(f['depth_sup'], (n,)) if t != L.LOSS_RGB_ONLY else None)
        n_out = L.LEVEL_PARAMS + (1 if bad_count is not None else 0)
        grads = out if out is not None else torch.empty(n_out, device=self.device)
        if grads.numel() < n_out or not grads.is_contiguous() or grads.dtype != torch.float32:
            raise L.NerfppError('backward(): `out` needs %d contiguous float32 elements' % n_out)
        a = L.BackwardArgs()
        a.n_rays, a.n_samples, a.precision = n, S, self.bwd_precision
        a.workspace_precision = self.precision
        a.ray_d, a.fg_far, a.fg_z, a.bg_z = [t.data_ptr() for t in (ray_d, fg_far, fg_z, bg_z)]
        a.packed, a.workspace, a.tables = self.packed_bwd.data_ptr(), self.workspace.data_ptr(), self.tables.data_ptr()
        if fused_loss is None:
            a.g_rgb, a.g_depth = g_rgb.data_ptr(), g_depth.data_ptr()
            a.g_fg_weights = g_fg_weights.data_ptr() if g_fg_weights is not None else None
        else:
            a.fused_loss, a.loss_type = 1, t
            a.lambda_depth, a.kl_sigma = float(fused_loss.get('lambda_depth', 1.0)), float(fused_loss.get('kl_sigma', 0.01))
            a.rgb, a.depth, a.rgb_gt = keep[0].data_ptr(), keep[1].data_ptr(), keep[2].data_ptr()
            a.depth_sup = keep[3].data_ptr() if keep[3] is not None else None
        a.grad_scale = float(grad_scale)
        a.grads = grads.data_ptr()
        a.params = self.params.data_ptr()
        if events is not None:
            a.ev_bwd_begin, a.ev_bwd_end, a.ev_dw_begin, a.ev_dw_end = [e.cuda_event for e in events]
        a.defer_reduce = int(bool(defer_reduce))
        if bad_count is not None:
            if bad_count.dtype != torch.int32 or bad_count.numel() != 1 or bad_count.device != self.device:
                raise L.NerfppError('bad_count: one int32 on the engine\'s device')
            a.bad_count = bad_count.data_ptr()
        L.check(L.lib().nerfpp_level_backward(_stream(), C.byref(a)), 'nerfpp_level_backward')
        self._bwd_args = (a, grads, bad_count, torch.cuda.current_stream()) if defer_reduce else None
        return grads

    def reduce_grads(self):
        if getattr(self, '_bwd_args', None) is None:
            raise L.NerfppError('reduce_grads() needs a preceding backward(defer_reduce=True)')
        a, grads, bad_count, bwd_stream = self._bwd_args
        self._bwd_args = None
        st = torch.cuda.current_stream()
        if bad_count is not None and st != bwd_stream:
            bad_count.record_stream(st)
        L.check(L.lib().nerfpp_level_reduce_grads(_stream(), C.byref(a)), 'nerfpp_level_reduce_grads')
        return grads


def loss_and_grads(ret, rgb_gt, depth_sup=None, loss_type='rgbonly', lambda_depth=1.0, kl_sigma=0.01,
                   fg_z_vals=None, fg_far_depth=None):
    rgb = _f32(ret['rgb'])
    n = rgb.shape[0]
    S = ret['fg_weights'].shape[1]
    dev = rgb.device
    t = L.LOSS_TYPES[loss_type]
    scalars = torch.empty(4, device=dev)
    g_rgb = torch.empty(n, 3, device=dev)
    g_depth = torch.empty(n, device=dev)
    g_w = torch.empty(n, S, device=dev) if t == L.LOSS_KL else None
    rgb_gt = _f32(rgb_gt, (n, 3))
    depth_sup = _f32(depth_sup, (n,)) if depth_sup is not None else None
    fg_z_vals = _f32(fg_z_vals) if fg_z_vals is not None else None
    fg_far_depth = _f32(fg_far_depth) if fg_far_depth is not None else None
    L.check(L.lib().nerfpp_loss(_stream(), n, S, t, float(lambda_depth), float(kl_sigma), _p(rgb), _p(rgb_gt),
                                _p(_f32(ret['depth'])), _p(depth_sup), _p(_f32(ret['fg_weights'])), _p(fg_z_vals),
                                _p(_f32(ret['fg_dists'])), _p(fg_far_depth), _p(scalars), _p(g_rgb), _p(g_depth),
                                _p(g_w)), 'nerfpp_loss')
    return scalars, g_rgb, g_depth, g_w


def adam_step(params, grads, exp_avg, exp_avg_sq, step, lr=5e-4, beta1=0.9, beta2=0.999, eps=1e-8, skip=None):
    if skip is not None and (skip.dtype != torch.float32 or not skip.is_cuda):
        raise L.NerfppError('adam_step: skip must be a float32 device tensor')
    L.check(L.lib().nerfpp_adam_step(_stream(), _p(params), _p(grads), _p(exp_avg), _p(exp_avg_sq),
                                     params.numel(), int(step), lr, beta1, beta2, eps, _p(skip)), 'nerfpp_adam_step')
```

outdoor_nerf_depth_amd/trainer.py:

```python
import os

import numpy as np
import torch

from . import _lib as L
from . import depth_losses as DL
from . import ops
from .model import init_level_params

ALGO_MACS = {
    'fwd': (593408, 604160),
    'dx': (557696, 557696),
}


class NerfppTrainer(object):
    def __init__(self, device, precision=L.PREC_SPLIT_BF16, cascade_samples=(64, 128), lrate=5e-4,
                 use_depth=True, depth_loss_type='mse', lambda_depth=0.1, depth_sigma=0.01, depth_scale=1.0,
                 world_size=1, level_params=None, overlap_allreduce=True, optim_autoexpo=False, img_names=None,
                 lambda_autoexpo=1.0, seed=777, torch_rng=False, fuse_loss=False, comm=None, depth_ssi_min_rays=8):
        self.device = torch.device(device)
        self.comm = comm
        self.precision = precision
        self.cascade_samples = tuple(cascade_samples)
        self.lrate = lrate
        self.loss_type = depth_loss_type if use_depth else 'rgbonly'
        if self.loss_type not in DL.names('nerfpp'):
            raise ValueError("depth_loss_type %r: only mse / l1 / kl exist in the reference "
                             "('los' and 'nll' are dead code there); ssi is this implementation's, and so is gnll" % depth_loss_type)
        row = DL.LOSSES[self.loss_type]
        self.ssi_min_rays = int(depth_ssi_min_rays)
        if 'min_rays' in row.extra and self.ssi_min_rays < 1:
            raise ValueError("depth_loss_type %r: depth_ssi_min_rays = %r, expected at least 1" % (self.loss_type, depth_ssi_min_rays))
        self.last_gnll_stats = None
        for flag, name in ((fuse_loss, 'fuse_loss'), (optim_autoexpo, 'optim_autoexpo')):
            if flag and name in row.refuses:
                raise ValueError("depth_loss_type %r and %s cannot be combined: %s" % (self.loss_type, name, DL.REFUSAL[name]))
        self.lambda_depth = lambda_depth
        self.kl_sigma = depth_sigma * depth_scale
        self.world_size = world_size
        if level_params is None:
            level_params = init_level_params(len(self.cascade_samples))
        self.engines = [ops.LevelEngine(p.to(self.device), precision) for p in level_params]
        self.exp_avg = [torch.zeros_like(e.params) for e in self.engines]
        self.exp_avg_sq = [torch.zeros_like(e.params) for e in self.engines]
        self.grads = [torch.zeros(L.LEVEL_PARAMS + 4, device=self.device) for _ in self.engines]
        self.step_count = 0
        self.seed, self.torch_rng = int(seed), bool(torch_rng)
        self.fuse_loss = bool(fuse_loss)
        self.rng_step = 0
        self.bad_cameras = torch.zeros(1, dtype=torch.int32, device=self.device)
        self.autoexpo = None
        if optim_autoexpo:
            if not img_names:
                raise ValueError('optim_autoexpo needs the training image names (ddp_model.py:168)')
            from .autoexpo import AutoExposure
            self.img_names = list(img_names)
            self.autoexpo = [AutoExposure(img_names, self.device, lrate, lambda_autoexpo, world_size)
                             for _ in self.engines]
        self._ae_grad = [None] * len(self.engines)
        self.last_autoexpo = [None] * len(self.engines)
        self.update_stream = torch.cuda.Stream(device=self.device) if overlap_allreduce else None
        self.level_streams = [torch.cuda.Stream(device=self.device) for _ in range(len(self.cascade_samples))] if overlap_allreduce else None
        self.concurrent_backward = True
        self._pending = {}
        self.wait_taps = None
        self.comm_taps = None

    def _update(self, m, step):
        eng = self.engines[m]
        eng.reduce_grads()
        flag = self.grads[m][L.LEVEL_PARAMS:L.LEVEL_PARAMS + 1]
        if self.world_size > 1 or self.comm is not None:
            import torch.distributed as dist
            if self.autoexpo is not None:
                if self._ae_grad[m] is None:
                    self._ae_grad[m] = torch.zeros(len(self.autoexpo[m].names), 3, device=self.device)
                if self.comm is not None:
                    self.comm.allreduce_mean(self._ae_grad[m].view(-1), prescaled=True)
                else:
                    dist.all_reduce(self._ae_grad[m])
            tap = None
            if self.comm_taps is not None:
                tap = (torch.cuda.Event(enable_timing=True), torch.cuda.Event(enable_timing=True))
                tap[0].record()
            if self.comm is not None:
                self.comm.allreduce_mean(self.grads[m], prescaled=True)
            else:
                dist.all_reduce(self.grads[m])
            if tap is not None:
                tap[1].record()
                self.comm_taps.append((m, tap[0], tap[1]))
        ops.adam_step(eng.params, self.grads[m][:L.LEVEL_PARAMS], self.exp_avg[m], self.exp_avg_sq[m], step, lr=self.lrate,
                      skip=flag)
        eng.repack()
        if self._ae_grad[m] is not None:
            self.autoexpo[m].apply(self._ae_grad[m][:, :2], self._ae_grad[m][:, 2] > 0)
            self._ae_grad[m] = None

    def _update_begin(self, m):
        if self.update_stream is None:
            self._update(m, self.step_count)
            return
        ev = torch.cuda.Event()
        ev.record()
        self.update_stream.wait_event(ev)
        if self._ae_grad[m] is not None:
            self._ae_grad[m].record_stream(self.update_stream)
        with torch.cuda.stream(self.update_stream):
            self._update(m, self.step_count)
            done = torch.cuda.Event()
            done.record()
        self._pending[m] = done

    def _update_end(self, m):
        done = self._pending.pop(m, None)
        if done is not None:
            if self.wait_taps is not None:
                a, b = torch.cuda.Event(enable_timing=True), torch.cuda.Event(enable_timing=True)
                a.record()
                torch.cuda.current_stream().wait_event(done)
                b.record()
                self.wait_taps.append((a, b))
            else:
                torch.cuda.current_stream().wait_event(done)

    def flush(self):
        for m in list(self._pending):
            self._update_end(m)

    def check_cameras(self):
        bad = int(self.bad_cameras.item())
        if self.world_size > 1 and self.step_count > 0:
            self.flush()
            bad += int(sum(float(g[L.LEVEL_PARAMS].item()) for g in self.grads))
        if bad != 0:
            self.bad_cameras.zero_()
            for g in self.grads:
                g[L.LEVEL_PARAMS:].zero_()
            raise Exception(ops.CAMERA_ERROR)

    def train_step(self, batch, uniforms=None, events=None):
        self.step_count += 1
        ray_o, ray_d = batch['ray_o'], batch['ray_d']
        n = ray_o.shape[0]
        S0, S1 = self.cascade_samples[0], self.cascade_samples[1] if len(self.cascade_samples) > 1 else 0
        dev = self.device
        u = uniforms or {}
        self.rng_step += 1
        rng = None if (uniforms is not None or self.torch_rng) else (self.seed, self.rng_step)
        if rng is not None:
            far, fg_z, bg_z = ops.sample_coarse(ray_o, ray_d, batch['min_depth'], S0, check=False, rng=rng,
                                                bad=self.bad_cameras)
        else:
            t_fg = u['t_fg'] if 't_fg' in u else torch.rand(n, S0, device=dev)
            t_bg = u['t_bg'] if 't_bg' in u else torch.rand(n, S0, device=dev)
            far, fg_z, bg_z = ops.sample_coarse(ray_o, ray_d, batch['min_depth'], S0, t_fg, t_bg, check=False,
                                                bad=self.bad_cameras)
        depth_sup = batch.get('depth_sup') if self.loss_type != 'rgbonly' else None
        row = DL.LOSSES[self.loss_type]
        scalars = []
        ret = None
        ae_idx = None
        if self.autoexpo is not None:
            name = batch.get('img_name')
            if name is None and 'frame' in batch:
                name = self.img_names[int(batch['frame'])]
            ae_idx = self.autoexpo[0].lookup(name)
        for m, eng in enumerate(self.engines):
            self._update_end(m)
            if m > 0 and rng is not None:
                fg_z, bg_z = ops.sample_fine_pair(fg_z, ret['fg_weights'], bg_z, ret['bg_weights'], S1, rng=rng)
            elif m > 0:
                u_fg = u['u_fg'] if 'u_fg' in u else torch.rand(n, S1, device=dev)
                u_bg = u['u_bg'] if 'u_bg' in u else torch.rand(n, S1, device=dev)
                fg_z, bg_z = ops.sample_fine_pair(fg_z, ret['fg_weights'], bg_z, ret['bg_weights'], S1,
                                                  u_fg=u_fg, u_bg=u_bg)
            ev = events[m] if events is not None else None
            ret = eng.forward(ray_o, ray_d, far, fg_z, bg_z, training=True,
                              events=ev['fwd'] if ev else None)
            ae = self.autoexpo[m] if ae_idx is not None else None
            if ae is None and self.fuse_loss:
                loss_done = None
                if self.update_stream is not None:
                    fwd_done = torch.cuda.Event()
                    fwd_done.record()
                    self.update_stream.wait_event(fwd_done)
                    with torch.cuda.stream(self.update_stream):
                        sc = ops.loss_and_grads(ret, batch['rgb'], depth_sup, self.loss_type, self.lambda_depth,
                                                self.kl_sigma, fg_z, far)[0]
                        loss_done = torch.cuda.Event()
                        loss_done.record()
                eng.backward(None, None, None, grad_scale=1.0 / self.world_size, out=self.grads[m][:L.LEVEL_PARAMS + 1], bad_count=self.bad_cameras,
                             events=ev['bwd'] if ev else None, defer_reduce=True,
                             fused_loss=dict(loss_type=self.loss_type, lambda_depth=self.lambda_depth, kl_sigma=self.kl_sigma,
                                             ret=ret, rgb_gt=batch['rgb'], depth_sup=depth_sup))
                if loss_done is not None:
                    torch.cuda.current_stream().wait_event(loss_done)
                else:
                    sc = ops.loss_and_grads(ret, batch['rgb'], depth_sup, self.loss_type, self.lambda_depth,
                                            self.kl_sigma, fg_z, far)[0]
                scalars.append(sc)
                self._update_begin(m)
                continue
            rgb_gt = ae.target(ae_idx, batch['rgb']) if ae is not None else batch['rgb']
            if row.nerfpp == DL.AFTER:
                for key in ('depth_sup', 'depth_std'):
                    if (key == 'depth_sup' or key in row.inputs) and batch.get(key) is None:
                        raise L.NerfppError("depth_loss_type %r: the batch has no %s" % (self.loss_type, key))
                sc, g_rgb, g_depth, g_w = ops.loss_and_grads(ret, rgb_gt, None, 'rgbonly', self.lambda_depth)
                if 'weights' in row.reads:
                    g_w = torch.zeros_like(ret['fg_weights'])
                _, stats = DL.after(self.loss_type, dict(weights=[ret['fg_weights']], x=[fg_z], pred=[ret['depth']]), depth_sup,
                                    [self.lambda_depth], dict(weights=[g_w], pred=[g_depth]),
                                    dict(total=sc[0:1], last=sc[2:3], n_sup=sc[3:4]),
                                    dict(min_rays=self.ssi_min_rays, norm='supervised', prior_std=batch.get('depth_std'), limit=far))
                if row.stats is not None and hasattr(self, row.stats):
                    setattr(self, row.stats, (getattr(self, row.stats) if m > 0 else []) + [stats])
            else:
                sc, g_rgb, g_depth, g_w = ops.loss_and_grads(ret, rgb_gt, depth_sup, self.loss_type,
                                                             self.lambda_depth, self.kl_sigma, fg_z, far)
            if ae is not None:
                g_ae = ae.finish(ae_idx, ret['rgb'], batch['rgb'], sc, g_rgb, self.lambda_depth)
                rows = torch.zeros(len(ae.names), 3, device=dev)
                rows[ae_idx, :2] = g_ae
                rows[ae_idx, 2] = 1.0
                self._ae_grad[m] = rows
                self.last_autoexpo[m] = ae.scale_shift(ae_idx)
            if self.concurrent_backward and m + 1 < len(self.engines) and ae is None and events is None and self.update_stream is not None:
                stream = self.level_streams[m]
                fwd_done = torch.cuda.Event()
                fwd_done.record()
                stream.wait_event(fwd_done)
                for t in [g_rgb, g_depth, g_w, ray_o, ray_d, far, fg_z, bg_z, batch['rgb'], depth_sup] + list(ret.values()):
                    if torch.is_tensor(t):
                        t.record_stream(stream)
                with torch.cuda.stream(stream):
                    eng.backward(g_rgb, g_depth, g_w, grad_scale=1.0 / self.world_size, out=self.grads[m][:L.LEVEL_PARAMS + 1], bad_count=self.bad_cameras,
                                 defer_reduce=True)
                    self._update_begin(m)
                scalars.append(sc)
                continue
            eng.backward(g_rgb, g_depth, g_w, grad_scale=1.0 / self.world_size, out=self.grads[m][:L.LEVEL_PARAMS + 1], bad_count=self.bad_cameras,
                         events=ev['bwd'] if ev else None, defer_reduce=True)
            scalars.append(sc)
            self._update_begin(m)
        return scalars


def batch_to_device(b, device):
    out = {}
    for k, v in b.items():
        if isinstance(v, np.ndarray):
            out[k] = torch.from_numpy(np.ascontiguousarray(v)).to(device)
    return out
```

Measured before the change: 486,300.

## Fuse composite forward, loss head and composite backward into one ray-side kernel

Adds a fused forward entry point that runs a single ray-side kernel after the MLP. It composites the ray, computes the loss gradients and writes the per-sample output gradients (d_out) directly into the training workspace. The backward pass can then skip its own composite_bwd launch via a DOUT_READY mode, so the raw MLP outputs are not re-read and the volume rendering is not recomputed. The trainer enables this path by default (fuse_loss=None) and runs the scalar loss on a side stream. This adds branching in the trainer and more register pressure in the combined kernel.

```diff
diff --git a/include/nerfpp_hip.h b/include/nerfpp_hip.h
--- a/include/nerfpp_hip.h
+++ b/include/nerfpp_hip.h
@@ -26,6 +26,9 @@
 #define NERFPP_LOSS_L1 2
 #define NERFPP_LOSS_KL 3
 
+#define NERFPP_FUSED_LOSS 1
+#define NERFPP_DOUT_READY 2
+
 #define NERFPP_FG_PARAMS 595844
 #define NERFPP_BG_PARAMS 606596
 #define NERFPP_LEVEL_PARAMS 1202440
@@ -91,6 +94,7 @@
 
 int64_t nerfpp_workspace_bytes(int n_rays, int n_samples, int precision, int training);
 
+#define NERFPP_WS_D_OUT 30
 int nerfpp_workspace_tensor(int n_rays, int n_samples, int precision, int net, int tensor,
                             int64_t* byte_offset, int32_t* ld, int64_t* plane_bytes);
 
@@ -119,6 +123,19 @@
 } nerfpp_forward_args;
 
 int nerfpp_level_forward(void* stream, const nerfpp_forward_args* args);
+
+#define NERFPP_RAY_SIDE_REVISION 1
+int nerfpp_ray_side_revision(void);
+
+typedef struct {
+  int32_t loss_type;
+  float lambda_depth;
+  float kl_sigma;
+  const float* rgb_gt;
+  const float* depth_sup;
+} nerfpp_loss_head_args;
+
+int nerfpp_level_forward_fused(void* stream, const nerfpp_forward_args* args, const nerfpp_loss_head_args* loss);
 
 int nerfpp_loss(void* stream, int n_rays, int n_samples, int loss_type, float lambda_depth,
                 float kl_sigma, const float* rgb, const float* rgb_gt, const float* depth,
diff --git a/outdoor_nerf_depth_amd/_lib.py b/outdoor_nerf_depth_amd/_lib.py
--- a/outdoor_nerf_depth_amd/_lib.py
+++ b/outdoor_nerf_depth_amd/_lib.py
@@ -28,6 +28,16 @@
                                    'rgb', 'depth', 'fg_weights', 'bg_weights', 'fg_dists', 'fg_rgb',
                                    'fg_depth', 'bg_rgb', 'bg_depth', 'bg_lambda', 'ev_mlp_begin',
                                    'ev_mlp_end')]
+
+
+class LossHeadArgs(C.Structure):
+    _fields_ = [('loss_type', C.c_int32), ('lambda_depth', C.c_float), ('kl_sigma', C.c_float),
+                ('rgb_gt', _fp), ('depth_sup', _fp)]
+
+
+FUSED_LOSS, DOUT_READY = 1, 2
+RAY_SIDE_REVISION = 1
+WS_D_OUT = 30
 
 
 class BackwardArgs(C.Structure):
@@ -67,6 +77,8 @@
     'nerfpp_workspace_bytes': (C.c_int64, [C.c_int, C.c_int, C.c_int, C.c_int]),
     'nerfpp_workspace_tensor': (C.c_int, [C.c_int, C.c_int, C.c_int, C.c_int, C.c_int, _i64p, _i32p, _i64p]),
     'nerfpp_level_forward': (C.c_int, [_fp, C.POINTER(ForwardArgs)]),
+    'nerfpp_ray_side_revision': (C.c_int, []),
+    'nerfpp_level_forward_fused': (C.c_int, [_fp, C.POINTER(ForwardArgs), C.POINTER(LossHeadArgs)]),
     'nerfpp_loss': (C.c_int, [_fp, C.c_int, C.c_int, C.c_int, C.c_float, C.c_float] + [_fp] * 12),
     'nerfpp_level_backward': (C.c_int, [_fp, C.POINTER(BackwardArgs)]),
     'nerfpp_level_reduce_grads': (C.c_int, [_fp, C.POINTER(BackwardArgs)]),
diff --git a/outdoor_nerf_depth_amd/csrc/nerfpp_api.hip b/outdoor_nerf_depth_amd/csrc/nerfpp_api.hip
--- a/outdoor_nerf_depth_amd/csrc/nerfpp_api.hip
+++ b/outdoor_nerf_depth_amd/csrc/nerfpp_api.hip
@@ -267,8 +267,15 @@
 int nerfpp_workspace_tensor(int n_rays, int n_samples, int precision, int net, int tensor, int64_t* byte_offset,
                             int32_t* ld, int64_t* plane_bytes) {
   REQUIRE(n_rays > 0 && n_samples >= 2 && n_samples <= NERFPP_MAX_SAMPLES && prec_ok_fwd(precision), "sizes / precision");
+  REQUIRE(byte_offset && ld && plane_bytes, "non-null outputs");
+  if (net >= 0 && net < N_NET && tensor == NERFPP_WS_D_OUT) {
+    const WsLayout L = ws_layout(n_rays, n_samples, precision, true);
+    *byte_offset = (int64_t)L.d_out[net];
+    *ld = 4;
+    *plane_bytes = (int64_t)L.rows_padded * 16;
+    return NERFPP_OK;
+  }
   REQUIRE(net >= 0 && net < N_NET && tensor >= 0 && tensor < T_COUNT && tensor != T_R && tensor != T_DR, "net / tensor id");
-  REQUIRE(byte_offset && ld && plane_bytes, "non-null outputs");
   if (tensor == T_H0 && h0_recomputed(precision))
     return fail(NERFPP_ERR_UNSUPPORTED, "nerfpp_workspace_tensor: H0 is not materialised at precision %d (its weight-gradient job recomputes it from X)", precision);
   if (tensor == T_DZ0 + 7 && h0_recomputed(precision))
@@ -281,8 +288,20 @@
   return NERFPP_OK;
 }
 
-int nerfpp_level_forward(void* stream, const nerfpp_forward_args* a) {
+}
+
+static int nerfpp_level_forward_impl(void* stream, const nerfpp_forward_args* a, const nerfpp_loss_head_args* lh) {
   REQUIRE(a, "args");
+  LossFuse lf{};
+  if (lh) {
+    REQUIRE(a->training != 0, "the fused ray side writes the per-sample gradients to a training workspace: training != 0");
+    REQUIRE(lh->loss_type >= NERFPP_LOSS_RGB_ONLY && lh->loss_type <= NERFPP_LOSS_KL, "loss_type in 0..3");
+    REQUIRE(lh->rgb_gt, "fused loss head needs rgb_gt");
+    if (lh->loss_type != NERFPP_LOSS_RGB_ONLY) REQUIRE(lh->depth_sup, "fused depth loss needs depth_sup");
+    if (lh->loss_type == NERFPP_LOSS_KL) REQUIRE(lh->kl_sigma > 0.f, "kl_sigma > 0");
+    lf.type = lh->loss_type; lf.lambda_depth = lh->lambda_depth; lf.kl_sigma = lh->kl_sigma;
+    lf.rgb_gt = lh->rgb_gt; lf.depth_sup = lh->depth_sup;
+  }
   REQUIRE(a->n_rays > 0 && a->n_samples >= 2 && a->n_samples <= NERFPP_MAX_SAMPLES, "sizes");
   REQUIRE(prec_ok_fwd(a->precision), "precision must be 1, 2 or 3");
   REQUIRE(a->ray_o && a->ray_d && a->fg_far && a->fg_z && a->bg_z && a->packed && a->workspace, "inputs");
@@ -321,11 +340,30 @@
     launch_mlp_fwd_pair(st, P, train, mm[0], mm[1], 0);
   }
   if (a->ev_mlp_end) (void)hipEventRecord((hipEvent_t)a->ev_mlp_end, st);
+  if (lh) {
+    const CompositeOut out{a->rgb, a->depth, a->fg_weights, a->bg_weights, a->fg_dists, a->fg_rgb, a->fg_depth, a->bg_rgb,
+                           a->bg_depth, a->bg_lambda};
+    launch_ray_side(st, a->n_rays, a->n_samples, (const float*)(ws + L.out_raw[0]), (const float*)(ws + L.out_raw[1]),
+                    (const float*)(ws + L.depth_real), a->ray_d, a->fg_far, a->fg_z, a->bg_z, out,
+                    (float*)(ws + L.d_out[0]), (float*)(ws + L.d_out[1]), lf);
+    return check_launch("level_forward_fused");
+  }
   launch_composite_fwd(st, a->n_rays, a->n_samples, (const float*)(ws + L.out_raw[0]),
                        (const float*)(ws + L.out_raw[1]), (const float*)(ws + L.depth_real), a->ray_d, a->fg_far,
                        a->fg_z, a->bg_z, a->rgb, a->depth, a->fg_weights, a->bg_weights, a->fg_dists, a->fg_rgb,
                        a->fg_depth, a->bg_rgb, a->bg_depth, a->bg_lambda);
   return check_launch("level_forward");
+}
+
+extern "C" {
+
+int nerfpp_ray_side_revision(void) { return NERFPP_RAY_SIDE_REVISION; }
+
+int nerfpp_level_forward(void* stream, const nerfpp_forward_args* a) { return nerfpp_level_forward_impl(stream, a, nullptr); }
+
+int nerfpp_level_forward_fused(void* stream, const nerfpp_forward_args* a, const nerfpp_loss_head_args* lh) {
+  REQUIRE(lh, "loss head args");
+  return nerfpp_level_forward_impl(stream, a, lh);
 }
 
 int nerfpp_loss(void* stream, int n_rays, int n_samples, int loss_type, float lambda_depth, float kl_sigma,
@@ -411,7 +449,9 @@
   REQUIRE(a->ray_d && a->fg_far && a->fg_z && a->bg_z && a->packed && a->workspace && a->tables, "inputs");
   REQUIRE(a->grads && a->params, "gradients / params");
   LossFuse lf{};
-  if (a->fused_loss) {
+  const bool dout_ready = a->fused_loss == NERFPP_DOUT_READY;
+  if (dout_ready) {
+  } else if (a->fused_loss) {
     REQUIRE(a->loss_type >= NERFPP_LOSS_RGB_ONLY && a->loss_type <= NERFPP_LOSS_KL, "loss_type in 0..3");
     REQUIRE(a->rgb && a->rgb_gt, "fused loss head needs rgb and rgb_gt");
     if (a->loss_type != NERFPP_LOSS_RGB_ONLY) REQUIRE(a->depth && a->depth_sup, "fused depth loss needs depth and depth_sup");
@@ -430,10 +470,11 @@
   const TblLayout T = tbl_layout();
   char* ws = (char*)a->workspace;
   const char* pk = (const char*)a->packed;
-  launch_composite_bwd(st, a->n_rays, a->n_samples, (const float*)(ws + L.out_raw[0]),
-                       (const float*)(ws + L.out_raw[1]), (const float*)(ws + L.depth_real), a->ray_d, a->fg_far,
-                       a->fg_z, a->bg_z, a->g_rgb, a->g_depth, a->g_fg_weights, (float*)(ws + L.d_out[0]),
-                       (float*)(ws + L.d_out[1]), a->fused_loss ? &lf : nullptr);
+  if (!dout_ready)
+    launch_composite_bwd(st, a->n_rays, a->n_samples, (const float*)(ws + L.out_raw[0]),
+                         (const float*)(ws + L.out_raw[1]), (const float*)(ws + L.depth_real), a->ray_d, a->fg_far,
+                         a->fg_z, a->bg_z, a->g_rgb, a->g_depth, a->g_fg_weights, (float*)(ws + L.d_out[0]),
+                         (float*)(ws + L.d_out[1]), a->fused_loss ? &lf : nullptr);
   MlpBwdArgs mb[N_NET];
   for (int net = 0; net < N_NET; ++net) {
     MlpBwdArgs& m = mb[net];
diff --git a/outdoor_nerf_depth_amd/csrc/nerfpp_kernels.h b/outdoor_nerf_depth_amd/csrc/nerfpp_kernels.h
--- a/outdoor_nerf_depth_amd/csrc/nerfpp_kernels.h
+++ b/outdoor_nerf_depth_amd/csrc/nerfpp_kernels.h
@@ -47,6 +47,10 @@
   const float* depth_sup;
 };
 
+struct CompositeOut {
+  float *rgb, *depth, *fg_weights, *bg_weights, *fg_dists, *fg_rgb, *fg_depth, *bg_rgb, *bg_depth, *bg_lambda;
+};
+
 struct DwArgs {
   NetWs ws[N_NET];
   int64_t rows, rows_padded;
@@ -81,6 +85,9 @@
                           const float* depth_real_bg, const float* ray_d, const float* fg_far,
                           const float* fg_z, const float* bg_z, const float* g_rgb, const float* g_depth,
                           const float* g_fg_weights, float* dout_fg, float* dout_bg, const nerfpp::LossFuse* lf);
+void launch_ray_side(hipStream_t st, int n, int S, const float* raw_fg, const float* raw_bg, const float* depth_real_bg,
+                     const float* ray_d, const float* fg_far, const float* fg_z, const float* bg_z,
+                     const nerfpp::CompositeOut& out, float* dout_fg, float* dout_bg, const nerfpp::LossFuse& lf);
 void launch_loss(hipStream_t st, int n, int S, int type, float lambda_depth, float kl_sigma, const float* rgb,
                  const float* rgb_gt, const float* depth, const float* depth_sup, const float* fg_weights,
                  const float* fg_z, const float* fg_dists, const float* fg_far, float* scalars, float* g_rgb,
diff --git a/outdoor_nerf_depth_amd/csrc/nerfpp_render.hip b/outdoor_nerf_depth_amd/csrc/nerfpp_render.hip
--- a/outdoor_nerf_depth_amd/csrc/nerfpp_render.hip
+++ b/outdoor_nerf_depth_amd/csrc/nerfpp_render.hip
@@ -322,55 +322,64 @@
   }
 }
 
-__global__ __launch_bounds__(256) void composite_fwd_kernel(
-    int n, int S, const float4* __restrict__ raw_fg, const float4* __restrict__ raw_bg,
-    const float* __restrict__ depth_real_bg, const float* __restrict__ ray_d,
-    const float* __restrict__ fg_far, const float* __restrict__ fg_z, const float* __restrict__ bg_z,
-    float* __restrict__ rgb, float* __restrict__ depth, float* __restrict__ fg_weights,
-    float* __restrict__ bg_weights, float* __restrict__ fg_dists, float* __restrict__ fg_rgb,
-    float* __restrict__ fg_depth, float* __restrict__ bg_rgb, float* __restrict__ bg_depth,
-    float* __restrict__ bg_lambda) {
+struct RayInputs {
+  const float4* __restrict__ raw_fg; const float4* __restrict__ raw_bg;
+  const float* __restrict__ depth_real_bg; const float* __restrict__ ray_d; const float* __restrict__ fg_far;
+  const float* __restrict__ fg_z; const float* __restrict__ bg_z;
+};
+
+__device__ __forceinline__ void composite_ray_forward(RaySamples& vf, RaySamples& vb, int S, int cpl, int lane, int ray,
+                                                      size_t row0, const RayInputs& in, float dnorm,
+                                                      const CompositeOut& o, float rgb[3], float* depth) {
+  load_volume<false>(vf, S, cpl, lane, row0, in.raw_fg, in.fg_z + row0, nullptr, dnorm, in.fg_far[ray]);
+  float a0 = 0, a1 = 0, a2 = 0, ad = 0;
+#pragma unroll
+  for (int k = 0; k < CPL_MAX; ++k) {
+    const int i = lane * cpl + k;
+    if (k < cpl && i < S) {
+      o.fg_weights[row0 + i] = vf.w[k];
+      o.fg_dists[row0 + i] = vf.dist[k];
+      a0 += vf.w[k] * vf.c[k][0]; a1 += vf.w[k] * vf.c[k][1]; a2 += vf.w[k] * vf.c[k][2];
+      ad += vf.w[k] * vf.zval[k];
+    }
+  }
+  const float f0 = wave_sum(a0), f1 = wave_sum(a1), f2 = wave_sum(a2), fd = wave_sum(ad);
+  const float lam = vf.lambda;
+  load_volume<true>(vb, S, cpl, lane, row0, in.raw_bg, in.bg_z + row0, in.depth_real_bg, dnorm, 0.f);
+  a0 = a1 = a2 = ad = 0;
+#pragma unroll
+  for (int k = 0; k < CPL_MAX; ++k) {
+    const int i = lane * cpl + k;
+    if (k < cpl && i < S) {
+      o.bg_weights[row0 + i] = vb.w[k];
+      a0 += vb.w[k] * vb.c[k][0]; a1 += vb.w[k] * vb.c[k][1]; a2 += vb.w[k] * vb.c[k][2];
+      ad += vb.w[k] * vb.zval[k];
+    }
+  }
+  const float b0 = lam * wave_sum(a0), b1 = lam * wave_sum(a1), b2 = lam * wave_sum(a2);
+  const float bd = lam * wave_sum(ad);
+  rgb[0] = f0 + b0; rgb[1] = f1 + b1; rgb[2] = f2 + b2;
+  *depth = fd + bd;
+  if (lane == 0) {
+    o.fg_rgb[ray * 3] = f0; o.fg_rgb[ray * 3 + 1] = f1; o.fg_rgb[ray * 3 + 2] = f2;
+    o.bg_rgb[ray * 3] = b0; o.bg_rgb[ray * 3 + 1] = b1; o.bg_rgb[ray * 3 + 2] = b2;
+    o.rgb[ray * 3] = rgb[0]; o.rgb[ray * 3 + 1] = rgb[1]; o.rgb[ray * 3 + 2] = rgb[2];
+    o.fg_depth[ray] = fd; o.bg_depth[ray] = bd; o.depth[ray] = *depth; o.bg_lambda[ray] = lam;
+  }
+}
+
+__device__ __forceinline__ float ray_dir_norm(const float* __restrict__ ray_d, int ray) {
+  const float dx = ray_d[ray * 3], dy = ray_d[ray * 3 + 1], dz = ray_d[ray * 3 + 2];
+  return sqrtf(sum3(dx * dx, dy * dy, dz * dz));
+}
+
+__global__ __launch_bounds__(256) void composite_fwd_kernel(int n, int S, RayInputs in, CompositeOut out) {
   const int wave = threadIdx.x >> 6, lane = threadIdx.x & 63;
   const int ray = blockIdx.x * 4 + wave;
   if (ray >= n) return;
-  const int cpl = (S + 63) / 64;
-  const size_t row0 = (size_t)ray * S;
-  const float dx = ray_d[ray * 3], dy = ray_d[ray * 3 + 1], dz = ray_d[ray * 3 + 2];
-  const float dnorm = sqrtf(sum3(dx * dx, dy * dy, dz * dz));
-  RaySamples v;
-  load_volume<false>(v, S, cpl, lane, row0, raw_fg, fg_z + row0, nullptr, dnorm, fg_far[ray]);
-  float a0 = 0, a1 = 0, a2 = 0, ad = 0;
-#pragma unroll
-  for (int k = 0; k < CPL_MAX; ++k) {
-    const int i = lane * cpl + k;
-    if (k < cpl && i < S) {
-      fg_weights[row0 + i] = v.w[k];
-      fg_dists[row0 + i] = v.dist[k];
-      a0 += v.w[k] * v.c[k][0]; a1 += v.w[k] * v.c[k][1]; a2 += v.w[k] * v.c[k][2];
-      ad += v.w[k] * v.zval[k];
-    }
-  }
-  const float f0 = wave_sum(a0), f1 = wave_sum(a1), f2 = wave_sum(a2), fd = wave_sum(ad);
-  const float lam = v.lambda;
-  load_volume<true>(v, S, cpl, lane, row0, raw_bg, bg_z + row0, depth_real_bg, dnorm, 0.f);
-  a0 = a1 = a2 = ad = 0;
-#pragma unroll
-  for (int k = 0; k < CPL_MAX; ++k) {
-    const int i = lane * cpl + k;
-    if (k < cpl && i < S) {
-      bg_weights[row0 + i] = v.w[k];
-      a0 += v.w[k] * v.c[k][0]; a1 += v.w[k] * v.c[k][1]; a2 += v.w[k] * v.c[k][2];
-      ad += v.w[k] * v.zval[k];
-    }
-  }
-  const float b0 = lam * wave_sum(a0), b1 = lam * wave_sum(a1), b2 = lam * wave_sum(a2);
-  const float bd = lam * wave_sum(ad);
-  if (lane == 0) {
-    fg_rgb[ray * 3] = f0; fg_rgb[ray * 3 + 1] = f1; fg_rgb[ray * 3 + 2] = f2;
-    bg_rgb[ray * 3] = b0; bg_rgb[ray * 3 + 1] = b1; bg_rgb[ray * 3 + 2] = b2;
-    rgb[ray * 3] = f0 + b0; rgb[ray * 3 + 1] = f1 + b1; rgb[ray * 3 + 2] = f2 + b2;
-    fg_depth[ray] = fd; bg_depth[ray] = bd; depth[ray] = fd + bd; bg_lambda[ray] = lam;
-  }
+  RaySamples vf, vb;
+  float rgb[3], depth;
+  composite_ray_forward(vf, vb, S, (S + 63) / 64, lane, ray, (size_t)ray * S, in, ray_dir_norm(in.ray_d, ray), out, rgb, &depth);
 }
 
 struct KlFuse { bool on; float gt, inv2s, lambda_depth; };
@@ -415,17 +424,9 @@
   }
 }
 
-template <bool LF>
-__global__ __launch_bounds__(256) void composite_bwd_kernel(
-    int n, int S, const float4* __restrict__ raw_fg, const float4* __restrict__ raw_bg,
-    const float* __restrict__ depth_real_bg, const float* __restrict__ ray_d,
-    const float* __restrict__ fg_far, const float* __restrict__ fg_z, const float* __restrict__ bg_z,
-    const float* __restrict__ g_rgb, const float* __restrict__ g_depth,
-    const float* __restrict__ g_fg_weights, float4* __restrict__ dout_fg, float4* __restrict__ dout_bg, LossFuse lf) {
-  const int wave = threadIdx.x >> 6, lane = threadIdx.x & 63;
-  const int ray = blockIdx.x * 4 + wave;
+__device__ __forceinline__ float loss_head_count(const LossFuse& lf, int n, int wave, int lane) {
   float cnt = 0.f;
-  if (LF && (lf.type == 1 || lf.type == 2)) {
+  if (lf.type == 1 || lf.type == 2) {
     __shared__ float s_cnt[4];
     float c = 0.f;
     for (int r = threadIdx.x; r < n; r += 256) c += lf.depth_sup[r] > 0.f ? 1.f : 0.f;
@@ -434,50 +435,89 @@
     __syncthreads();
     cnt = (s_cnt[0] + s_cnt[1]) + (s_cnt[2] + s_cnt[3]);
   }
+  return cnt;
+}
+
+__device__ __forceinline__ void loss_head_grads(const LossFuse& lf, int n, int ray, float cnt, const float rgb[3], float depth,
+                                                float far, float gC[3], float* gD, KlFuse* kl) {
+#pragma unroll
+  for (int c = 0; c < 3; ++c) gC[c] = 2.f * (rgb[c] - lf.rgb_gt[ray * 3 + c]) / (float)(3 * n);
+  *gD = 0.f;
+  if (lf.type == 1 || lf.type == 2) {
+    const float gt = lf.depth_sup[ray];
+    if (gt > 0.f && cnt > 0.f) {
+      const float d = depth - gt;
+      *gD = lf.type == 1 ? lf.lambda_depth * 2.f * d / cnt
+                         : lf.lambda_depth * (d > 0.f ? 1.f : (d < 0.f ? -1.f : 0.f)) / cnt;
+    }
+  } else if (lf.type == 3) {
+    const float gt = lf.depth_sup[ray];
+    kl->on = gt > 0.f && gt < far;
+    kl->gt = gt;
+    kl->inv2s = 1.f / (2.f * lf.kl_sigma);
+    kl->lambda_depth = lf.lambda_depth;
+  }
+}
+
+__device__ __forceinline__ void composite_ray_backward(const RaySamples& vf, const RaySamples& vb, int S, int cpl, int lane,
+                                                       size_t row0, const float gC[3], float gD,
+                                                       const float* __restrict__ g_fg_weights, float4* __restrict__ dout_fg,
+                                                       float4* __restrict__ dout_bg, const KlFuse kl) {
+  float a0 = 0, a1 = 0, a2 = 0, ad = 0;
+#pragma unroll
+  for (int k = 0; k < CPL_MAX; ++k) {
+    a0 += vb.w[k] * vb.c[k][0]; a1 += vb.w[k] * vb.c[k][1]; a2 += vb.w[k] * vb.c[k][2];
+    ad += vb.w[k] * vb.zval[k];
+  }
+  const float g_lam = gC[0] * wave_sum(a0) + gC[1] * wave_sum(a1) + gC[2] * wave_sum(a2) + gD * wave_sum(ad);
+  const float lam = vf.lambda;
+  volume_backward<false>(vf, S, cpl, lane, row0, gC, gD, g_lam * lam, g_fg_weights, dout_fg, kl);
+  const float gCb[3] = {lam * gC[0], lam * gC[1], lam * gC[2]};
+  volume_backward<true>(vb, S, cpl, lane, row0, gCb, lam * gD, 0.f, nullptr, dout_bg);
+}
+
+template <bool LF>
+__global__ __launch_bounds__(256) void composite_bwd_kernel(
+    int n, int S, RayInputs in, const float* __restrict__ g_rgb, const float* __restrict__ g_depth,
+    const float* __restrict__ g_fg_weights, float4* __restrict__ dout_fg, float4* __restrict__ dout_bg, LossFuse lf) {
+  const int wave = threadIdx.x >> 6, lane = threadIdx.x & 63;
+  const int ray = blockIdx.x * 4 + wave;
+  const float cnt = LF ? loss_head_count(lf, n, wave, lane) : 0.f;
   if (ray >= n) return;
   const int cpl = (S + 63) / 64;
   const size_t row0 = (size_t)ray * S;
-  const float dx = ray_d[ray * 3], dy = ray_d[ray * 3 + 1], dz = ray_d[ray * 3 + 2];
-  const float dnorm = sqrtf(sum3(dx * dx, dy * dy, dz * dz));
+  const float dnorm = ray_dir_norm(in.ray_d, ray);
   float gC[3], gD;
   KlFuse kl{false, 0.f, 0.f, 0.f};
   if (LF) {
-#pragma unroll
-    for (int c = 0; c < 3; ++c) gC[c] = 2.f * (lf.rgb[ray * 3 + c] - lf.rgb_gt[ray * 3 + c]) / (float)(3 * n);
-    gD = 0.f;
-    if (lf.type == 1 || lf.type == 2) {
-      const float gt = lf.depth_sup[ray];
-      if (gt > 0.f && cnt > 0.f) {
-        const float d = lf.depth[ray] - gt;
-        gD = lf.type == 1 ? lf.lambda_depth * 2.f * d / cnt
-                          : lf.lambda_depth * (d > 0.f ? 1.f : (d < 0.f ? -1.f : 0.f)) / cnt;
-      }
-    } else if (lf.type == 3) {
-      const float gt = lf.depth_sup[ray];
-      kl.on = gt > 0.f && gt < fg_far[ray];
-      kl.gt = gt;
-      kl.inv2s = 1.f / (2.f * lf.kl_sigma);
-      kl.lambda_depth = lf.lambda_depth;
-    }
+    const float rgb[3] = {lf.rgb[ray * 3], lf.rgb[ray * 3 + 1], lf.rgb[ray * 3 + 2]};
+    const float depth = (lf.type == 1 || lf.type == 2) ? lf.depth[ray] : 0.f;
+    loss_head_grads(lf, n, ray, cnt, rgb, depth, in.fg_far[ray], gC, &gD, &kl);
   } else {
     gC[0] = g_rgb[ray * 3]; gC[1] = g_rgb[ray * 3 + 1]; gC[2] = g_rgb[ray * 3 + 2];
     gD = g_depth[ray];
   }
-  RaySamples vb;
-  load_volume<true>(vb, S, cpl, lane, row0, raw_bg, bg_z + row0, depth_real_bg, dnorm, 0.f);
-  float a0 = 0, a1 = 0, a2 = 0, ad = 0;
-#pragma unroll
-  for (int k = 0; k < CPL_MAX; ++k) {
-    a0 += vb.w[k] * vb.c[k][0]; a1 += vb.w[k] * vb.c[k][1]; a2 += vb.w[k] * vb.c[k][2];
-    ad += vb.w[k] * vb.zval[k];
-  }
-  const float g_lam = gC[0] * wave_sum(a0) + gC[1] * wave_sum(a1) + gC[2] * wave_sum(a2) + gD * wave_sum(ad);
-  RaySamples vf;
-  load_volume<false>(vf, S, cpl, lane, row0, raw_fg, fg_z + row0, nullptr, dnorm, fg_far[ray]);
-  const float lam = vf.lambda;
-  volume_backward<false>(vf, S, cpl, lane, row0, gC, gD, g_lam * lam, LF ? nullptr : g_fg_weights, dout_fg, kl);
-  const float gCb[3] = {lam * gC[0], lam * gC[1], lam * gC[2]};
-  volume_backward<true>(vb, S, cpl, lane, row0, gCb, lam * gD, 0.f, nullptr, dout_bg);
+  RaySamples vb, vf;
+  load_volume<true>(vb, S, cpl, lane, row0, in.raw_bg, in.bg_z + row0, in.depth_real_bg, dnorm, 0.f);
+  load_volume<false>(vf, S, cpl, lane, row0, in.raw_fg, in.fg_z + row0, nullptr, dnorm, in.fg_far[ray]);
+  composite_ray_backward(vf, vb, S, cpl, lane, row0, gC, gD, LF ? nullptr : g_fg_weights, dout_fg, dout_bg, kl);
+}
+
+__global__ __launch_bounds__(256) void ray_side_kernel(int n, int S, RayInputs in, CompositeOut out,
+                                                       float4* __restrict__ dout_fg, float4* __restrict__ dout_bg,
+                                                       LossFuse lf) {
+  const int wave = threadIdx.x >> 6, lane = threadIdx.x & 63;
+  const int ray = blockIdx.x * 4 + wave;
+  const float cnt = loss_head_count(lf, n, wave, lane);
+  if (ray >= n) return;
+  const int cpl = (S + 63) / 64;
+  const size_t row0 = (size_t)ray * S;
+  RaySamples vf, vb;
+  float rgb[3], depth, gC[3], gD;
+  composite_ray_forward(vf, vb, S, cpl, lane, ray, row0, in, ray_dir_norm(in.ray_d, ray), out, rgb, &depth);
+  KlFuse kl{false, 0.f, 0.f, 0.f};
+  loss_head_grads(lf, n, ray, cnt, rgb, depth, in.fg_far[ray], gC, &gD, &kl);
+  composite_ray_backward(vf, vb, S, cpl, lane, row0, gC, gD, nullptr, dout_fg, dout_bg, kl);
 }
 
 __device__ double block_sum(double v, double (&sh)[1][1024]) {
@@ -614,21 +654,26 @@
                           const float* fg_z, const float* bg_z, float* rgb, float* depth, float* fg_weights,
                           float* bg_weights, float* fg_dists, float* fg_rgb, float* fg_depth, float* bg_rgb,
                           float* bg_depth, float* bg_lambda) {
-  hipLaunchKernelGGL(composite_fwd_kernel, dim3((n + 3) / 4), dim3(256), 0, st, n, S, (const float4*)raw_fg,
-                     (const float4*)raw_bg, depth_real_bg, ray_d, fg_far, fg_z, bg_z, rgb, depth, fg_weights,
-                     bg_weights, fg_dists, fg_rgb, fg_depth, bg_rgb, bg_depth, bg_lambda);
+  const RayInputs in{(const float4*)raw_fg, (const float4*)raw_bg, depth_real_bg, ray_d, fg_far, fg_z, bg_z};
+  const CompositeOut out{rgb, depth, fg_weights, bg_weights, fg_dists, fg_rgb, fg_depth, bg_rgb, bg_depth, bg_lambda};
+  hipLaunchKernelGGL(composite_fwd_kernel, dim3((n + 3) / 4), dim3(256), 0, st, n, S, in, out);
+}
+void launch_ray_side(hipStream_t st, int n, int S, const float* raw_fg, const float* raw_bg, const float* depth_real_bg,
+                     const float* ray_d, const float* fg_far, const float* fg_z, const float* bg_z,
+                     const nerfpp::CompositeOut& out, float* dout_fg, float* dout_bg, const nerfpp::LossFuse& lf) {
+  const RayInputs in{(const float4*)raw_fg, (const float4*)raw_bg, depth_real_bg, ray_d, fg_far, fg_z, bg_z};
+  hipLaunchKernelGGL(ray_side_kernel, dim3((n + 3) / 4), dim3(256), 0, st, n, S, in, out, (float4*)dout_fg, (float4*)dout_bg, lf);
 }
 void launch_composite_bwd(hipStream_t st, int n, int S, const float* raw_fg, const float* raw_bg,
                           const float* depth_real_bg, const float* ray_d, const float* fg_far,
                           const float* fg_z, const float* bg_z, const float* g_rgb, const float* g_depth,
                           const float* g_fg_weights, float* dout_fg, float* dout_bg, const nerfpp::LossFuse* lf) {
+  const RayInputs in{(const float4*)raw_fg, (const float4*)raw_bg, depth_real_bg, ray_d, fg_far, fg_z, bg_z};
   if (lf)
-    hipLaunchKernelGGL(composite_bwd_kernel<true>, dim3((n + 3) / 4), dim3(256), 0, st, n, S, (const float4*)raw_fg,
-                       (const float4*)raw_bg, depth_real_bg, ray_d, fg_far, fg_z, bg_z, g_rgb, g_depth,
+    hipLaunchKernelGGL(composite_bwd_kernel<true>, dim3((n + 3) / 4), dim3(256), 0, st, n, S, in, g_rgb, g_depth,
                        g_fg_weights, (float4*)dout_fg, (float4*)dout_bg, *lf);
   else
-    hipLaunchKernelGGL(composite_bwd_kernel<false>, dim3((n + 3) / 4), dim3(256), 0, st, n, S, (const float4*)raw_fg,
-                       (const float4*)raw_bg, depth_real_bg, ray_d, fg_far, fg_z, bg_z, g_rgb, g_depth,
+    hipLaunchKernelGGL(composite_bwd_kernel<false>, dim3((n + 3) / 4), dim3(256), 0, st, n, S, in, g_rgb, g_depth,
                        g_fg_weights, (float4*)dout_fg, (float4*)dout_bg, nerfpp::LossFuse{});
 }
 void launch_loss(hipStream_t st, int n, int S, int type, float lambda_depth, float kl_sigma, const float* rgb,
diff --git a/outdoor_nerf_depth_amd/ops.py b/outdoor_nerf_depth_amd/ops.py
--- a/outdoor_nerf_depth_amd/ops.py
+++ b/outdoor_nerf_depth_amd/ops.py
@@ -198,7 +198,7 @@
             self.workspace = torch.empty(need, dtype=torch.uint8, device=self.device)
         return self.workspace
 
-    def forward(self, ray_o, ray_d, fg_z_max, fg_z_vals, bg_z_vals, training=False, events=None):
+    def forward(self, ray_o, ray_d, fg_z_max, fg_z_vals, bg_z_vals, training=False, events=None, loss_head=None):
         ray_o, ray_d = _f32(ray_o), _f32(ray_d)
         n = ray_o.shape[0]
         fg_z_vals = _f32(fg_z_vals)
@@ -221,7 +221,19 @@
             setattr(a, k, out[k].data_ptr())
         if events is not None:
             a.ev_mlp_begin, a.ev_mlp_end = events[0].cuda_event, events[1].cuda_event
-        L.check(L.lib().nerfpp_level_forward(_stream(), C.byref(a)), 'nerfpp_level_forward')
+        if loss_head is not None:
+            if not training:
+                raise L.NerfppError('forward(loss_head=...) needs training=True')
+            h = L.LossHeadArgs()
+            h.loss_type = L.LOSS_TYPES[loss_head['loss_type']]
+            h.lambda_depth, h.kl_sigma = float(loss_head.get('lambda_depth', 1.0)), float(loss_head.get('kl_sigma', 0.01))
+            rgb_gt = _f32(loss_head['rgb_gt'], (n, 3))
+            depth_sup = _f32(loss_head['depth_sup'], (n,)) if h.loss_type != L.LOSS_RGB_ONLY else None
+            h.rgb_gt, h.depth_sup = rgb_gt.data_ptr(), (depth_sup.data_ptr() if depth_sup is not None else None)
+            L.check(L.lib().nerfpp_level_forward_fused(_stream(), C.byref(a), C.byref(h)), 'nerfpp_level_forward_fused')
+        else:
+            L.check(L.lib().nerfpp_level_forward(_stream(), C.byref(a)), 'nerfpp_level_forward')
+        self._dout_ready = loss_head is not None
         if training:
             self._fwd = (n, S, ray_d, fg_z_max, fg_z_vals, bg_z_vals)
         return out
@@ -241,13 +253,26 @@
         blk = blk.view(rows_p // 32, ld // 16, 32, 2, 2, 4).permute(0, 2, 1, 4, 3, 5)
         return blk.reshape(rows_p, ld)[:rows].float()
 
+    def d_out(self, net):
+        if self._fwd is None:
+            raise L.NerfppError('d_out() needs a preceding forward(training=True)')
+        n, S = self._fwd[0], self._fwd[1]
+        off, ld, pb = C.c_int64(), C.c_int32(), C.c_int64()
+        L.check(L.lib().nerfpp_workspace_tensor(n, S, self.precision, int(net), L.WS_D_OUT, C.byref(off), C.byref(ld),
+                                                C.byref(pb)), 'nerfpp_workspace_tensor')
+        return self.workspace[off.value: off.value + n * S * 16].view(torch.float32).view(n * S, 4)
+
     def backward(self, g_rgb, g_depth, g_fg_weights=None, grad_scale=1.0, out=None, events=None, defer_reduce=False,
-                 fused_loss=None, bad_count=None):
+                 fused_loss=None, bad_count=None, dout_ready=False):
         if self._fwd is None:
             raise L.NerfppError('backward() needs a preceding forward(training=True)')
         n, S, ray_d, fg_far, fg_z, bg_z = self._fwd
         keep = None
-        if fused_loss is None:
+        if dout_ready:
+            if not getattr(self, '_dout_ready', False):
+                raise L.NerfppError('backward(dout_ready=True) needs a preceding forward(training=True, loss_head=...)')
+            g_rgb = g_depth = g_fg_weights = fused_loss = None
+        elif fused_loss is None:
             g_rgb, g_depth = _f32(g_rgb, (n, 3)), _f32(g_depth, (n,))
             g_fg_weights = _f32(g_fg_weights, (n, S)) if g_fg_weights is not None else None
         else:
@@ -265,7 +290,9 @@
         a.workspace_precision = self.precision
         a.ray_d, a.fg_far, a.fg_z, a.bg_z = [t.data_ptr() for t in (ray_d, fg_far, fg_z, bg_z)]
         a.packed, a.workspace, a.tables = self.packed_bwd.data_ptr(), self.workspace.data_ptr(), self.tables.data_ptr()
-        if fused_loss is None:
+        if dout_ready:
+            a.fused_loss = L.DOUT_READY
+        elif fused_loss is None:
             a.g_rgb, a.g_depth = g_rgb.data_ptr(), g_depth.data_ptr()
             a.g_fg_weights = g_fg_weights.data_ptr() if g_fg_weights is not None else None
         else:
diff --git a/outdoor_nerf_depth_amd/trainer.py b/outdoor_nerf_depth_amd/trainer.py
--- a/outdoor_nerf_depth_amd/trainer.py
+++ b/outdoor_nerf_depth_amd/trainer.py
@@ -18,7 +18,7 @@
     def __init__(self, device, precision=L.PREC_SPLIT_BF16, cascade_samples=(64, 128), lrate=5e-4,
                  use_depth=True, depth_loss_type='mse', lambda_depth=0.1, depth_sigma=0.01, depth_scale=1.0,
                  world_size=1, level_params=None, overlap_allreduce=True, optim_autoexpo=False, img_names=None,
-                 lambda_autoexpo=1.0, seed=777, torch_rng=False, fuse_loss=False, comm=None, depth_ssi_min_rays=8):
+                 lambda_autoexpo=1.0, seed=777, torch_rng=False, fuse_loss=None, comm=None, depth_ssi_min_rays=8):
         self.device = torch.device(device)
         self.comm = comm
         self.precision = precision
@@ -48,6 +48,7 @@
         self.step_count = 0
         self.seed, self.torch_rng = int(seed), bool(torch_rng)
         self.fuse_loss = bool(fuse_loss)
+        self.ray_side = fuse_loss is None
         self.rng_step = 0
         self.bad_cameras = torch.zeros(1, dtype=torch.int32, device=self.device)
         self.autoexpo = None
@@ -160,6 +161,7 @@
         depth_sup = batch.get('depth_sup') if self.loss_type != 'rgbonly' else None
         row = DL.LOSSES[self.loss_type]
         scalars = []
+        side_losses = []
         ret = None
         ae_idx = None
         if self.autoexpo is not None:
@@ -177,9 +179,41 @@
                 fg_z, bg_z = ops.sample_fine_pair(fg_z, ret['fg_weights'], bg_z, ret['bg_weights'], S1,
                                                   u_fg=u_fg, u_bg=u_bg)
             ev = events[m] if events is not None else None
+            ae = self.autoexpo[m] if ae_idx is not None else None
+            if self.ray_side and ae is None and row.nerfpp != DL.AFTER and (depth_sup is not None or self.loss_type == 'rgbonly'):
+                ret = eng.forward(ray_o, ray_d, far, fg_z, bg_z, training=True, events=ev['fwd'] if ev else None,
+                                  loss_head=dict(loss_type=self.loss_type, lambda_depth=self.lambda_depth, kl_sigma=self.kl_sigma,
+                                                 rgb_gt=batch['rgb'], depth_sup=depth_sup))
+                fork = self.concurrent_backward and m + 1 < len(self.engines) and events is None and self.update_stream is not None
+                if self.update_stream is not None:
+                    fwd_done = torch.cuda.Event()
+                    fwd_done.record()
+                    self.update_stream.wait_event(fwd_done)
+                    with torch.cuda.stream(self.update_stream):
+                        sc = ops.loss_and_grads(ret, batch['rgb'], depth_sup, self.loss_type, self.lambda_depth,
+                                                self.kl_sigma, fg_z, far)[0]
+                        loss_done = torch.cuda.Event()
+                        loss_done.record()
+                    sc.record_stream(torch.cuda.current_stream())
+                    side_losses.append((loss_done, ret, fg_z, far))
+                if fork:
+                    stream = self.level_streams[m]
+                    stream.wait_event(fwd_done)
+                    with torch.cuda.stream(stream):
+                        eng.backward(None, None, grad_scale=1.0 / self.world_size, out=self.grads[m][:L.LEVEL_PARAMS + 1],
+                                     bad_count=self.bad_cameras, defer_reduce=True, dout_ready=True)
+                        self._update_begin(m)
+                else:
+                    eng.backward(None, None, grad_scale=1.0 / self.world_size, out=self.grads[m][:L.LEVEL_PARAMS + 1],
+                                 bad_count=self.bad_cameras, events=ev['bwd'] if ev else None, defer_reduce=True, dout_ready=True)
+                    if self.update_stream is None:
+                        sc = ops.loss_and_grads(ret, batch['rgb'], depth_sup, self.loss_type, self.lambda_depth,
+                                                self.kl_sigma, fg_z, far)[0]
+                    self._update_begin(m)
+                scalars.append(sc)
+                continue
             ret = eng.forward(ray_o, ray_d, far, fg_z, bg_z, training=True,
                               events=ev['fwd'] if ev else None)
-            ae = self.autoexpo[m] if ae_idx is not None else None
             if ae is None and self.fuse_loss:
                 loss_done = None
                 if self.update_stream is not None:
@@ -245,6 +279,8 @@
                          events=ev['bwd'] if ev else None, defer_reduce=True)
             scalars.append(sc)
             self._update_begin(m)
+        for done in side_losses:
+            torch.cuda.current_stream().wait_event(done[0])
         return scalars
 
 
```

New measurement: 483,900. About the same (-0.5%).
